# rockcarry/ffcnn

Measured on AMD Instinct MI355X. Metric: frames/sec yolo-fastest-1.1 @320x320 batch-64 per GPU (u8 BGR frames -> net_input's conversion in the first kernel -> full forward: conv stack + YOLO decode + NMS, boxes on rank 0), higher is better.
Workload: dtype f32

## Files before the change

ffcnn_amd/capi.py:

```python
import ctypes as C
import os
import subprocess

import numpy as np

HERE = os.path.dirname(os.path.abspath(__file__))
ROOT = os.path.dirname(HERE)
DATA = os.path.join(ROOT, "data")
CFG = os.path.join(DATA, "yolo-fastest-1.1.cfg")
WEIGHTS = os.path.join(DATA, "yolo-fastest-1.1.weights")

f32p = C.POINTER(C.c_float)


class FFGPU:
    MAX_DET = 128
    MERGE_LDS_SLOTS = 1024
    KEEP_ALL, COMPAT_V6, NO_GRAPH, NO_FUSE, HOST_DETS, SPLIT2, CONCURRENT, BF16_PW = 1, 2, 4, 8, 16, 32, 64, 128
    FEAT_FLAT, FEAT_MEAN, FEAT_MAX = 0, 1, 2
    POST_NONE, POST_SOFTMAX, POST_L2 = 0, 1, 2
    TOPK_MAX = 16
    RELABEL_KEEP_SCORE, RELABEL_LABEL_SCORE = 0, 1
    RELABEL_ENTRIES, RELABEL_MERGED = 0, 1
    K_AUTO, K_GENERIC, K_DW_STREAM, K_DW_LDS, K_PW_MFMA, K_PW_GEMM, _K6, K_DENSE_SMALL, K_IGEMM, K_PW_BF16, K_GROUP_THIN, K_PW_X3, K_CONV_X3, K_PW_X3T = range(14)
# ... 74 lines not shown


class Label(C.Structure):
    _fields_ = [("index", C.c_int), ("value", C.c_float)]


class RelabelSpec(C.Structure):
    _fields_ = [("min_value", C.c_float), ("type_base", C.c_int), ("score_mode", C.c_int), ("reserved", C.c_int)]


class Gallery(C.Structure):
    _fields_ = [("d_rows", C.c_void_p), ("d_ids", C.c_void_p), ("d_head", C.c_void_p), ("row_stride", C.c_long), ("capacity", C.c_int), ("d", C.c_int)]


class RedactSpec(C.Structure):
    _fields_ = [("mode", C.c_int), ("cell", C.c_int), ("flags", C.c_int), ("nclasses", C.c_int), ("classes", C.c_void_p), ("min_score", C.c_float),
                ("margin_num", C.c_int), ("margin_den", C.c_int), ("color", C.c_ubyte * 4)]


class Zone(C.Structure):
    _fields_ = [("x", C.c_float * 8), ("y", C.c_float * 8), ("nverts", C.c_int), ("dwell_frames", C.c_int), ("classes", C.c_uint * 4), ("reserved", C.c_int * 2)]


class Line(C.Structure):
    _fields_ = [("ax", C.c_float), ("ay", C.c_float), ("bx", C.c_float), ("by", C.c_float), ("classes", C.c_uint * 4)]


class Scene(C.Structure):
    _fields_ = [("zone", Zone * 8), ("line", Line * 8), ("nzones", C.c_int), ("nlines", C.c_int), ("anchor", C.c_int), ("reserved", C.c_int)]


class ZonesSpec(C.Structure):
    _fields_ = [("capacity", C.c_int), ("max_missed", C.c_int), ("identity", C.c_int), ("flags", C.c_int), ("min_score", C.c_float),
                ("gate_zone", C.c_uint), ("gate_line", C.c_uint), ("reserved", C.c_int)]


class ZoneSlot(C.Structure):
    _fields_ = [("id", C.c_int), ("px", C.c_float), ("py", C.c_float), ("inside", C.c_int), ("last", C.c_int), ("reserved", C.c_int * 3), ("since", C.c_int * 8)]


SCENE_ZONES, SCENE_LINES, ZONE_VERTS, ZONES_DETS, ZONES_ROW = 8, 8, 8, 128, 64
ZONES_NONE, ZONES_TYPE, ZONES_IDS = 0, 1, 2
ZONES_GATE_INVERT = 1
ZONES_ENTRIES, ZONES_MERGED = 0, 1
ZONES_EVENTS_HEADER = ("considered", "known", "fresh", "refused", "duplicate", "anonymous", "dropped", "freed", "live", "frame")
ZONES_STATE_HEADER = 144
TRACK_DETS = 128
TRACK_ENTRIES, TRACK_MERGED = 0, 1
TRACK_IDS_HEADER = ("considered", "matched", "born", "refused", "dropped", "freed", "live", "frame")
CROP_F32, CROP_U8 = 0, 1
CROP_ENTRIES, CROP_MERGED = 0, 1
REDACT_FILL, REDACT_MOSAIC = 0, 1
REDACT_OUTSIDE = 1
REDACT_ENTRIES, REDACT_MERGED = 0, 1
DRAW_ENTRIES, DRAW_MERGED = 0, 1
YUV_BT601_LIMITED, YUV_BT601_FULL, YUV_BT709_LIMITED, YUV_BT709_FULL = 0, 1, 2, 3

assert C.sizeof(LAYER) == 120 and C.sizeof(NET) == 104 and C.sizeof(BBOX) == 24
assert C.sizeof(FrameDets) == 16 + 24 * FFGPU.MAX_DET
assert C.sizeof(BgrFrame) == 24 and C.sizeof(Nv12Frame) == 40 and C.sizeof(Tile) == 16 and C.sizeof(TileRect) == 16
assert C.sizeof(DrawStyle) == 24 and C.sizeof(CropSpec) == 72 and C.sizeof(Crop) == 48
assert C.sizeof(TrackSpec) == 32 and C.sizeof(Track) == 48
assert C.sizeof(FeatureSpec) == 16 and C.sizeof(Label) == 8 and C.sizeof(RelabelSpec) == 16
assert C.sizeof(Gallery) == 40 and C.sizeof(RedactSpec) == 40
assert C.sizeof(Zone) == 96 and C.sizeof(Line) == 32 and C.sizeof(Scene) == 1040 and C.sizeof(ZonesSpec) == 32 and C.sizeof(ZoneSlot) == 64

BOX_DTYPE = np.dtype([("type", "<i4"), ("score", "<f4"), ("x1", "<f4"), ("y1", "<f4"), ("x2", "<f4"), ("y2", "<f4")])
DETS_DTYPE = np.dtype([("count", "<i4"), ("ncand", "<i4"), ("overflow", "<i4"), ("nfull", "<i4"),
                       ("box", BOX_DTYPE, (FFGPU.MAX_DET,))])
CROP_DTYPE = np.dtype([("target", "<i4"), ("box", "<i4"), ("type", "<i4"), ("score", "<f4"), ("x0", "<i4"), ("y0", "<i4"), ("w", "<i4"), ("h", "<i4"),
                       ("sw", "<i4"), ("sh", "<i4"), ("s1", "<i4"), ("s2", "<i4")])
TRACK_DTYPE = np.dtype([("id", "<i4"), ("type", "<i4"), ("score", "<f4"), ("x1", "<f4"), ("y1", "<f4"), ("x2", "<f4"), ("y2", "<f4"),
                        ("hits", "<i4"), ("missed", "<i4"), ("born", "<i4"), ("det", "<i4"), ("reserved", "<i4")])
ZONE_SLOT_DTYPE = np.dtype([("id", "<i4"), ("px", "<f4"), ("py", "<f4"), ("inside", "<i4"), ("last", "<i4"), ("reserved", "<i4", (3,)), ("since", "<i4", (8,))])
LABEL_DTYPE = np.dtype([("index", "<i4"), ("value", "<f4")])

EXPORTS = ["net_load", "net_free", "net_input", "net_forward", "net_dump", "net_profile", "groupconv",
           "ffgpu_device_count", "ffgpu_set_device", "ffgpu_last_error", "ffgpu_build_info",
           "ffgpu_net_weights_dev", "ffgpu_net_weights_commit",
           "ffgpu_exec_create", "ffgpu_exec_destroy", "ffgpu_exec_batch", "ffgpu_exec_arena_bytes",
           "ffgpu_exec_kernel_count", "ffgpu_exec_work_model", "ffgpu_exec_set_scale", "ffgpu_exec_forward_dev", "ffgpu_exec_forward_host",
           "ffgpu_exec_forward_bgr_dev", "ffgpu_exec_forward_bgr_frames_dev", "ffgpu_exec_forward_nv12_frames_dev", "ffgpu_exec_dets_dev", "ffgpu_exec_dets_host", "ffgpu_exec_set_ring", "ffgpu_exec_set_ring_strided", "ffgpu_exec_read_dets", "ffgpu_exec_read_layer", "ffgpu_exec_hash_layers",
           "ffgpu_exec_read_boxes", "ffgpu_exec_cand_capacity", "ffgpu_exec_graph_captures",
           "ffgpu_exec_profile", "ffgpu_exec_profile_steps", "ffgpu_exec_step_model", "ffgpu_groupconv_dev", "ffgpu_groupconv_kernel_name", "ffgpu_groupconv_time_dev", "ffgpu_irb_dev", "ffgpu_irb_plan_text", "ffgpu_irb_instantiations", "ffgpu_knobs_text", "ffgpu_dwpw_dev", "ffgpu_packed_records_bytes", "ffgpu_pack_records", "ffgpu_unpack_records",
           "ffgpu_shard_range", "ffgpu_node_create", "ffgpu_node_destroy", "ffgpu_node_ndev", "ffgpu_node_shard", "ffgpu_node_set_scale",
           "ffgpu_node_input_dev", "ffgpu_node_input_slot_dev", "ffgpu_node_depth", "ffgpu_node_rccl_ranks", "ffgpu_node_forward", "ffgpu_node_forward_host",
           "ffgpu_node_submit", "ffgpu_node_wait", "ffgpu_node_run",
           "ffgpu_merge_tiles_scratch_bytes", "ffgpu_merge_tiles_dev", "ffgpu_exec_merge_tiles", "ffgpu_exec_merged_dev", "ffgpu_exec_read_merged",
           "ffgpu_exec_read_merged_boxes", "ffgpu_tile_plan",
           "ffgpu_draw_boxes_bgr_dev", "ffgpu_draw_boxes_nv12_dev", "ffgpu_exec_draw_bgr", "ffgpu_exec_draw_nv12",
           "ffgpu_crop_table_bytes", "ffgpu_crop_slot_bytes", "ffgpu_crop_boxes_bgr_dev", "ffgpu_crop_boxes_nv12_dev", "ffgpu_exec_crop_bgr", "ffgpu_exec_crop_nv12",
           "ffgpu_crops_to_source_dev",
           "ffgpu_track_state_bytes", "ffgpu_track_reset_dev", "ffgpu_track_boxes_dev", "ffgpu_exec_track",
           "ffgpu_feature_dim", "ffgpu_exec_feature_dim", "ffgpu_features_dev", "ffgpu_exec_features", "ffgpu_topk_dev", "ffgpu_crops_relabel_dev",
           "ffgpu_exec_relabel",
           "ffgpu_match_workspace_bytes", "ffgpu_match_dev", "ffgpu_gallery_enroll_dev",
           "ffgpu_redact_boxes_bgr_dev", "ffgpu_redact_boxes_nv12_dev", "ffgpu_exec_redact_bgr", "ffgpu_exec_redact_nv12",
           "ffgpu_zones_state_bytes", "ffgpu_scene_check", "ffgpu_zones_reset_dev", "ffgpu_zones_boxes_dev", "ffgpu_exec_zones"]
DIAG_EXPORTS = ["ffgpu_membench", "ffgpu_pipe_probe", "ffgpu_pipe_probe2", "ffgpu_pipe_probe3", "ffgpu_mfma_floor", "ffgpu_diag_x3_term", "ffgpu_diag_xl_op", "ffgpu_clock_probe"]


def library_path():
    return os.environ.get("FFCNN_HIP_LIB") or os.path.join(HERE, "lib", "libffcnn_hip.so")


def build_library(force=False):
    cmd = ["make", "-C", os.path.join(HERE, "csrc")]
    if force:
        subprocess.check_call(cmd + ["clean"], stdout=subprocess.DEVNULL)
    subprocess.check_call(cmd, stdout=subprocess.DEVNULL)
    return library_path()


_lib = None


def lib():
    global _lib
    if _lib is not None:
        return _lib
    path = library_path()
    if not os.path.exists(path):
        raise RuntimeError("%s is missing: run `python -c 'import __graft_entry__ as g; g.build()'` "
                           "(the HIP extension is the only compute path)" % path)
    L = C.CDLL(path)
    vp, i, sz = C.c_void_p, C.c_int, C.c_size_t
    L.net_load.restype = C.POINTER(NET)
    L.net_load.argtypes = [C.c_char_p, C.c_char_p, i, i]
    L.net_free.argtypes = [C.POINTER(NET)]
    L.net_input.argtypes = [C.POINTER(NET), vp, i, i, f32p, f32p]
    L.net_forward.argtypes = [C.POINTER(NET)]
    L.net_dump.argtypes = [C.POINTER(NET)]
    L.net_profile.argtypes = [C.POINTER(NET)]
    L.groupconv.argtypes = [f32p, f32p, f32p] + [i] * 12 + [C.POINTER(f32p), C.POINTER(i)]
    L.ffgpu_last_error.restype = C.c_char_p
    L.ffgpu_build_info.restype = C.c_char_p
    if b" DIAG " in L.ffgpu_build_info() and os.environ.get("FFCNN_HIP_ALLOW_DIAG") != "1":
        raise RuntimeError("%s is a DIAG (lab) build of libffcnn_hip; set FFCNN_HIP_ALLOW_DIAG=1 to load it on purpose" % path)
    L.ffgpu_set_device.argtypes = [i]
    L.ffgpu_net_weights_dev.argtypes = [C.POINTER(NET), C.POINTER(vp), C.POINTER(sz)]
    L.ffgpu_net_weights_commit.argtypes = [C.POINTER(NET), vp]
    L.ffgpu_exec_create.restype = vp
    L.ffgpu_exec_create.argtypes = [C.POINTER(NET), i, i]
    L.ffgpu_exec_destroy.argtypes = [vp]
    L.ffgpu_exec_batch.argtypes = [vp]
    L.ffgpu_exec_arena_bytes.restype = sz
    L.ffgpu_exec_arena_bytes.argtypes = [vp]
    L.ffgpu_exec_kernel_count.argtypes = [vp]
    L.ffgpu_exec_work_model.argtypes = [vp, C.POINTER(C.c_double), C.POINTER(C.c_double)]
    L.ffgpu_exec_set_scale.argtypes = [vp, i, i]
    L.ffgpu_exec_forward_dev.argtypes = [vp, vp, vp]
    L.ffgpu_exec_forward_host.argtypes = [vp, f32p]
    L.ffgpu_exec_forward_bgr_dev.argtypes = [vp, vp, i, i, f32p, f32p, vp]
    L.ffgpu_exec_forward_bgr_frames_dev.argtypes = [vp, C.POINTER(BgrFrame), i, f32p, f32p, vp]
    L.ffgpu_exec_forward_nv12_frames_dev.argtypes = [vp, C.POINTER(Nv12Frame), i, f32p, f32p, vp]
    L.ffgpu_exec_dets_dev.argtypes = [vp, C.POINTER(vp), C.POINTER(sz)]
    L.ffgpu_exec_dets_host.restype = vp; L.ffgpu_exec_dets_host.argtypes = [vp]
    L.ffgpu_exec_set_ring.argtypes = [vp, vp, C.c_int]
    L.ffgpu_exec_set_ring_strided.argtypes = [vp, vp, C.c_int, C.c_int]
    L.ffgpu_exec_read_dets.argtypes = [vp, vp, i]
    L.ffgpu_exec_read_layer.argtypes = [vp, i, i, f32p, sz]
    L.ffgpu_exec_hash_layers.argtypes = [vp, vp, i]
    L.ffgpu_exec_profile.argtypes = [vp, vp, f32p]
    L.ffgpu_exec_profile_steps.argtypes = [vp, vp, C.POINTER(i), f32p, i]
    L.ffgpu_exec_step_model.argtypes = [vp, C.POINTER(i), C.POINTER(C.c_double), i]
    L.ffgpu_groupconv_dev.argtypes = [vp, vp, vp] + [i] * 15 + [vp]
    L.ffgpu_groupconv_kernel_name.restype = C.c_char_p
    L.ffgpu_groupconv_kernel_name.argtypes = [i] * 10
    L.ffgpu_groupconv_time_dev.restype = C.c_float
    L.ffgpu_groupconv_time_dev.argtypes = [vp, vp, vp] + [i] * 17 + [vp]
    L.ffgpu_irb_dev.restype = C.c_float
    L.ffgpu_irb_dev.argtypes = [vp] * 6 + [i] * 13 + [vp]
    L.ffgpu_irb_plan_text.argtypes = [i] * 12 + [C.c_char_p, i]
    L.ffgpu_irb_instantiations.argtypes = [C.c_char_p, i]
    L.ffgpu_knobs_text.argtypes = [C.c_char_p, i]
    L.ffgpu_exec_read_boxes.argtypes = [vp, i, vp, i]
    L.ffgpu_exec_cand_capacity.argtypes = [vp]
    L.ffgpu_exec_graph_captures.argtypes = [vp]
    L.ffgpu_dwpw_dev.restype = C.c_float
    L.ffgpu_dwpw_dev.argtypes = [vp] * 4 + [i] * 10 + [vp]
    L.ffgpu_packed_records_bytes.restype = C.c_size_t
    L.ffgpu_packed_records_bytes.argtypes = [i, i]
    L.ffgpu_pack_records.restype = i
    L.ffgpu_pack_records.argtypes = [vp, i, C.c_long, i, i, vp, vp]
    L.ffgpu_shard_range.argtypes = [i, i, i, C.POINTER(i), C.POINTER(i)]
    L.ffgpu_shard_range.restype = None
    L.ffgpu_node_create.restype = vp
    L.ffgpu_node_create.argtypes = [C.POINTER(NET), i, C.POINTER(i), i, i, i]
    L.ffgpu_node_destroy.argtypes = [vp]
    L.ffgpu_node_ndev.argtypes = [vp]
    L.ffgpu_node_shard.argtypes = [vp, i, C.POINTER(i), C.POINTER(i), C.POINTER(i)]
    L.ffgpu_node_set_scale.argtypes = [vp, i, i]
    L.ffgpu_node_input_dev.restype = vp
    L.ffgpu_node_input_dev.argtypes = [vp, i]
    L.ffgpu_node_input_slot_dev.restype = vp
    L.ffgpu_node_input_slot_dev.argtypes = [vp, i, i]
    L.ffgpu_node_depth.argtypes = [vp]
    if hasattr(L, "ffgpu_node_rccl_ranks"):
        L.ffgpu_node_rccl_ranks.argtypes = [vp]
    L.ffgpu_node_submit.restype = C.c_long
    L.ffgpu_node_submit.argtypes = [vp, f32p]
    L.ffgpu_node_wait.argtypes = [vp, C.c_long, vp]
    L.ffgpu_node_run.argtypes = [vp, C.c_long, vp]
    L.ffgpu_unpack_records.argtypes = [vp, i, i, vp]
    L.ffgpu_node_forward.argtypes = [vp, vp]
    L.ffgpu_node_forward_host.argtypes = [vp, f32p, vp]
    L.ffgpu_merge_tiles_scratch_bytes.restype = sz
    L.ffgpu_merge_tiles_scratch_bytes.argtypes = [i, i]
    L.ffgpu_merge_tiles_dev.argtypes = [vp, vp, i, C.POINTER(Tile), i, i, C.c_float, i, vp, vp, vp, sz, vp]
    L.ffgpu_exec_merge_tiles.argtypes = [vp, C.POINTER(Tile), i, i, vp]
    L.ffgpu_exec_merged_dev.argtypes = [vp, C.POINTER(vp), C.POINTER(sz)]
    L.ffgpu_exec_read_merged.argtypes = [vp, vp, i]
    L.ffgpu_exec_read_merged_boxes.argtypes = [vp, i, vp, i]
    L.ffgpu_tile_plan.argtypes = [i] * 7 + [C.POINTER(TileRect), i]
    L.ffgpu_draw_boxes_bgr_dev.argtypes = [vp, vp, i, C.POINTER(i), C.POINTER(BgrFrame), i, C.POINTER(DrawStyle), vp]
    L.ffgpu_draw_boxes_nv12_dev.argtypes = [vp, vp, i, C.POINTER(i), C.POINTER(Nv12Frame), i, C.POINTER(DrawStyle), vp]
    L.ffgpu_exec_draw_bgr.argtypes = [vp, i, C.POINTER(BgrFrame), i, C.POINTER(DrawStyle), vp]
    L.ffgpu_exec_draw_nv12.argtypes = [vp, i, C.POINTER(Nv12Frame), i, C.POINTER(DrawStyle), vp]
    L.ffgpu_redact_boxes_bgr_dev.argtypes = [vp, vp, i, C.POINTER(i), C.POINTER(BgrFrame), i, C.POINTER(RedactSpec), vp]
    L.ffgpu_redact_boxes_nv12_dev.argtypes = [vp, vp, i, C.POINTER(i), C.POINTER(Nv12Frame), i, C.POINTER(RedactSpec), vp]
    L.ffgpu_exec_redact_bgr.argtypes = [vp, i, C.POINTER(BgrFrame), i, C.POINTER(RedactSpec), vp]
    L.ffgpu_exec_redact_nv12.argtypes = [vp, i, C.POINTER(Nv12Frame), i, C.POINTER(RedactSpec), vp]
    L.ffgpu_crop_table_bytes.restype = sz
    L.ffgpu_crop_table_bytes.argtypes = [i]
    L.ffgpu_crop_slot_bytes.restype = sz
    L.ffgpu_crop_slot_bytes.argtypes = [i, i, i]
    L.ffgpu_crop_boxes_bgr_dev.argtypes = [vp, vp, i, C.POINTER(i), C.POINTER(BgrFrame), i, C.POINTER(CropSpec), vp, vp, i, vp]
    L.ffgpu_crop_boxes_nv12_dev.argtypes = [vp, vp, i, C.POINTER(i), C.POINTER(Nv12Frame), i, C.POINTER(CropSpec), vp, vp, i, vp]
    L.ffgpu_exec_crop_bgr.argtypes = [vp, i, C.POINTER(BgrFrame), i, C.POINTER(CropSpec), vp, vp, i, vp]
    L.ffgpu_exec_crop_nv12.argtypes = [vp, i, C.POINTER(Nv12Frame), i, C.POINTER(CropSpec), vp, vp, i, vp]
    L.ffgpu_crops_to_source_dev.argtypes = [vp, i, vp, vp, i, vp, vp, vp]
    L.ffgpu_track_state_bytes.restype = sz
    L.ffgpu_track_state_bytes.argtypes = [i, i]
    L.ffgpu_track_reset_dev.argtypes = [vp, i, i, i, vp]
    L.ffgpu_track_boxes_dev.argtypes = [vp, vp, i, C.POINTER(i), C.POINTER(i), i, C.POINTER(TrackSpec), vp, i, vp, vp, vp, vp]
    L.ffgpu_exec_track.argtypes = [vp, i, C.POINTER(i), i, C.POINTER(TrackSpec), vp, i, vp, vp, vp, vp]
    L.ffgpu_zones_state_bytes.restype = sz
    L.ffgpu_zones_state_bytes.argtypes = [i, i]
    L.ffgpu_scene_check.argtypes = [C.POINTER(Scene), i]
    L.ffgpu_zones_reset_dev.argtypes = [vp, i, i, i, vp]
    L.ffgpu_zones_boxes_dev.argtypes = [vp, vp, i, C.POINTER(i), C.POINTER(i), i, C.POINTER(ZonesSpec), vp, vp, i, vp, vp, vp, vp, vp]
    L.ffgpu_exec_zones.argtypes = [vp, i, C.POINTER(i), i, C.POINTER(ZonesSpec), vp, vp, i, vp, vp, vp, vp, vp]
    L.ffgpu_feature_dim.argtypes = [i, i, i, i]
    L.ffgpu_exec_feature_dim.argtypes = [vp, C.POINTER(FeatureSpec)]
    L.ffgpu_features_dev.argtypes = [vp, i, i, i, i, i, i, vp, C.c_long, vp]
    L.ffgpu_exec_features.argtypes = [vp, C.POINTER(FeatureSpec), vp, C.c_long, vp]
    L.ffgpu_topk_dev.argtypes = [vp, i, i, C.c_long, i, vp, vp]
    L.ffgpu_crops_relabel_dev.argtypes = [vp, i, vp, i, vp, vp, i, C.POINTER(i), i, C.POINTER(RelabelSpec), vp, vp, vp]
    L.ffgpu_exec_relabel.argtypes = [vp, i, vp, i, vp, i, i, C.POINTER(RelabelSpec), vp, vp, vp]
    L.ffgpu_match_workspace_bytes.restype = sz
    L.ffgpu_match_workspace_bytes.argtypes = [i, i, i]
    L.ffgpu_match_dev.argtypes = [vp, i, C.c_long, C.POINTER(Gallery), i, vp, vp, C.c_long, vp, sz, vp]
    L.ffgpu_gallery_enroll_dev.argtypes = [C.POINTER(Gallery), vp, i, C.c_long, vp, i, C.c_float, vp, vp]
    _lib = L
    return L

# ... 729 lines not shown
        _check(lib().ffgpu_node_run(self.h, steps, out.ctypes.data), "ffgpu_node_run")
        return out

    def input_slot_dev(self, rank, slot):
        return lib().ffgpu_node_input_slot_dev(self.h, rank, slot)

    def __init__(self, net, ndev, global_batch, devices=None, exec_flags=0, node_flags=0):
        self.net, self.ndev, self.total = net, ndev, global_batch
        dv = (C.c_int * ndev)(*devices) if devices is not None else None
        self.h = lib().ffgpu_node_create(net.p, ndev, dv, global_batch, exec_flags, node_flags)
        if not self.h:
            raise RuntimeError("ffgpu_node_create failed: %s" % last_error())

    def close(self):
        if self.h:
            lib().ffgpu_node_destroy(self.h)
            self.h = None

    def __enter__(self):
        return self

    def __exit__(self, *a):
        self.close()

    def shard(self, rank):
        lo, hi, dev = C.c_int(), C.c_int(), C.c_int()
        _check(lib().ffgpu_node_shard(self.h, rank, C.byref(lo), C.byref(hi), C.byref(dev)), "ffgpu_node_shard")
        return lo.value, hi.value, dev.value

    def set_scale(self, s1, s2):
        _check(lib().ffgpu_node_set_scale(self.h, s1, s2), "ffgpu_node_set_scale")

    def input_dev(self, rank):
        return lib().ffgpu_node_input_dev(self.h, rank)

    def forward(self):
        out = np.zeros(self.total, DETS_DTYPE)
        _check(lib().ffgpu_node_forward(self.h, out.ctypes.data), "ffgpu_node_forward")
        return out

    def forward_host(self, frames):
        frames = np.ascontiguousarray(frames, np.float32)
        assert frames.shape == (self.total,) + self.net.input_shape, frames.shape
        out = np.zeros(self.total, DETS_DTYPE)
        _check(lib().ffgpu_node_forward_host(self.h, frames.ctypes.data_as(f32p), out.ctypes.data), "ffgpu_node_forward_host")
        return out


def groupconv_dev(d_in, d_filt, d_out, batch, iw, ih, ic, groups, pad, stride, fs, fn, act=0, flags=0, variant=0, stream=None):
    ow, oh = (iw + 2 * pad - fs) // stride + 1, (ih + 2 * pad - fs) // stride + 1
    _check(lib().ffgpu_groupconv_dev(d_in, d_filt, d_out, batch, iw, ih, ic, groups, pad, stride, fs, fn, ow, oh, fn,
                                     act, flags, variant, stream), "ffgpu_groupconv_dev")


def groupconv_time_dev(d_in, d_filt, d_out, batch, iw, ih, ic, groups, pad, stride, fs, fn, act=0, flags=0, variant=0,
                       warmup=5, iters=20, stream=None):
    ow, oh = (iw + 2 * pad - fs) // stride + 1, (ih + 2 * pad - fs) // stride + 1
    us = lib().ffgpu_groupconv_time_dev(d_in, d_filt, d_out, batch, iw, ih, ic, groups, pad, stride, fs, fn, ow, oh, fn,
                                        act, flags, variant, warmup, iters, stream)
    if us < 0:
        raise RuntimeError("ffgpu_groupconv_time_dev failed: %s" % last_error())
    return us


def packed_records_bytes(batch, cap):
    return int(lib().ffgpu_packed_records_bytes(batch, cap))


def pack_records_dev(d_records, nslots, slot_stride_records, batch, cap, d_out, stream=None):
    _check(lib().ffgpu_pack_records(d_records, nslots, slot_stride_records, batch, cap, d_out, stream), "ffgpu_pack_records")


def kernel_name(batch, iw, ih, ic, groups, pad, stride, fs, fn, variant=0):
    return lib().ffgpu_groupconv_kernel_name(batch, iw, ih, ic, groups, pad, stride, fs, fn, variant).decode()


def irb_plan_text(shape, flags=0):
    buf = C.create_string_buffer(1024)
    if lib().ffgpu_irb_plan_text(*shape, flags, buf, len(buf)) < 0:
        raise RuntimeError("ffgpu_irb_plan_text failed: %s" % last_error())
    return buf.value.decode()


def irb_instantiations():
    buf = C.create_string_buffer(4096)
    n = lib().ffgpu_irb_instantiations(buf, len(buf))
    if n < 0 or n >= len(buf):
        raise RuntimeError("ffgpu_irb_instantiations failed: %s" % (last_error() if n < 0 else "%d bytes" % n))
    return buf.value.decode().split()


def knobs():
    buf = C.create_string_buffer(1 << 16)
    n = lib().ffgpu_knobs_text(buf, len(buf))
    if n < 0 or n >= len(buf):
        raise RuntimeError("ffgpu_knobs_text failed: %s" % (last_error() if n < 0 else "%d bytes" % n))
    rows = []
    for line in buf.value.decode().splitlines():
        name, kind, dflt, cls, value, text = line.split(" ", 5)
        rows.append({"name": name, "kind": kind, "default": None if dflt == "-" else dflt if dflt == "computed" else int(dflt), "cls": cls, "value": value, "text": text})
    return rows


def dwpw_dev(d_in, d_wd, d_wp, d_out, batch, iw, ih, c, oc, fs, actd=2, actp=0, warmup=0, iters=0, stream=None):
    us = lib().ffgpu_dwpw_dev(d_in, d_wd, d_wp, d_out, batch, iw, ih, c, oc, fs, actd, actp, warmup, iters, stream)
    if us < 0:
        raise RuntimeError("ffgpu_dwpw_dev failed: %s" % last_error())
    return us


def irb_dev(d_in, d_w1, d_wd, d_w2, d_res, d_out, batch, iw, ih, ic, ec, oc, stride, act1=2, actd=2, act2=0, res_act=0,
            warmup=0, iters=0, stream=None):
    us = lib().ffgpu_irb_dev(d_in, d_w1, d_wd, d_w2, d_res, d_out, batch, iw, ih, ic, ec, oc, stride, act1, actd, act2, res_act,
                             warmup, iters, stream)
    if us < 0:
        raise RuntimeError("ffgpu_irb_dev failed: %s" % last_error())
    return us
```

ffcnn_amd/csrc/ffgpu_conv_kernels.inc:

```
#include "ffgpu_dw_stream.inc"
#include "ffgpu_pw_mfma.inc"
#include "ffgpu_pw_gemm32.inc"
#include "ffgpu_pw_bf16.inc"
#include "ffgpu_conv_igemm.inc"
#include "ffgpu_dwpw.inc"
#include "ffgpu_conv_dense.inc"
#include "ffgpu_irb.inc"
#include "ffgpu_irb_thin.inc"
#include "ffgpu_front.inc"
#include "ffgpu_irb_wave.inc"
#include "ffgpu_irb_wave2.inc"
#include "ffgpu_pw_x3.inc"
#include "ffgpu_pw_x3t.inc"
#include "ffgpu_conv_x3.inc"
#include "ffgpu_dw_lds.inc"
#include "ffgpu_dw_pair.inc"
#include "ffgpu_conv_thin.inc"

struct BareScratch {
    float *p = nullptr; size_t n = 0; int dev = -1;
    float *get(size_t need)
    {
        int d = 0;
        (void)hipGetDevice(&d);
        if (p && dev == d && n >= need) return p;
        if (p) (void)hipFree(p);
        p = nullptr; n = 0; dev = d;
        if (hipMalloc(&p, need * sizeof(float)) != hipSuccess) { p = nullptr; return nullptr; }
        n = need;
        return p;
    }
};

static int device_cus()
{
    static int cu_of[64];
    static std::mutex cu_mu;
    int dev = 0, cus = 0;
    (void)hipGetDevice(&dev);
    std::lock_guard<std::mutex> lk(cu_mu);
    if (dev >= 0 && dev < 64) {
        if (!cu_of[dev]) (void)hipDeviceGetAttribute(&cu_of[dev], hipDeviceAttributeMultiprocessorCount, dev);
        cus = cu_of[dev];
    } else (void)hipDeviceGetAttribute(&cus, hipDeviceAttributeMultiprocessorCount, dev);
    return cus > 0 ? cus : 256;
}

static unsigned umulhi_magic(long dv) { return dv == 1 ? 0u : (unsigned)(((1ULL << 32) + (unsigned long long)dv - 1) / (unsigned long long)dv); }

static void split_main_narrow(long P, int ntm, int slots, bool narrow_on, long *ntn_main, long *ntn_narrow)
{
    const long ntn_all = (P + 127) / 128, total_all = ntn_all * ntm;
    long tail_tiles = total_all % slots;
    if (total_all <= slots / 2) tail_tiles = total_all;
    else if (tail_tiles > slots * 5 / 8) tail_tiles = 0;
    if (!narrow_on) tail_tiles = 0;
    const long tail_ntn = (tail_tiles + ntm - 1) / ntm;
    *ntn_main = ntn_all - tail_ntn;
    const long npx_narrow = P - *ntn_main * 128;
    *ntn_narrow = npx_narrow > 0 ? (npx_narrow + 63) / 64 : 0;
}

static bool conv_cnhw_contiguous(const ConvDesc &d)
{
    return d.in_ns == (long)d.iw * d.ih && d.in_cs == (long)d.N * d.iw * d.ih &&
           d.out_ns == (long)d.ow * d.oh && d.out_cs == (long)d.N * d.ow * d.oh &&
           (!d.residual || (d.res_ns == d.out_ns && d.res_cs == d.out_cs));
}
static bool conv_is_depthwise(const ConvDesc &d) { return d.groups == d.ic && d.ic == d.oc; }
static bool conv_is_pointwise(const ConvDesc &d) { return d.fs == 1 && d.stride == 1 && d.pad == 0 && d.groups == 1; }

static bool dw_stream_ok(const ConvDesc &d)
{
    return conv_is_depthwise(d) && d.fs == 3 && d.stride == 1 && d.pad == 1 && conv_cnhw_contiguous(d) &&
           d.iw % 4 == 0 && d.iw >= 40 && d.iw <= 512 && d.ih >= 2 && !d.residual && d.act != 3;
}
static bool pw_mfma_ok(const ConvDesc &d)
{
    const long P = (long)d.N * d.iw * d.ih;
    return conv_is_pointwise(d) && conv_cnhw_contiguous(d) && P % 4 == 0 && ((d.ic + 3) & ~3) <= 1024 && P < (1L << 28);
}

static int pw_x3_mt(const ConvDesc &d) { const int f = knob(K_PWX3_MT); return f == 4 || f == 2 || f == 1 ? f : 4; }
static bool pw_x3_ok(const ConvDesc &d)
{
    const long P = (long)d.N * d.iw * d.ih;
    return pw_mfma_ok(d) && (long)(d.ic + 32) * P < (1L << 30);
}
static bool pw_x3_auto(const ConvDesc &d)
{
    const long P = (long)d.N * d.iw * d.ih;
    return pw_x3_ok(d) && d.ic >= knob(K_PWX3_MIN_IC) && d.oc >= knob(K_PWX3_MIN_OC) && P >= knob(K_PWX3_MIN_P) &&
           knob(K_PW_X3) != 0;
}
// ... 1352 lines not shown
size_t ffgpu_irb_pack_floats(const IrbDesc &d) { return irb_planned(d, "irb_pack_floats") ? (size_t)d.plan.pack_floats : 0; }

int ffgpu_irb_pack(const IrbDesc &d, float *pk, hipStream_t s)
{
    const IrbPlan &c = d.plan;
    if (!irb_planned(d, "irb_pack")) return -1;
    if (c.family == IRB_THIN) return 0;
    if (c.family == IRB_WAVE) {
        IrbwPackP q; q.w1 = d.w1; q.wd = d.wd; q.w2 = d.w2; q.pk = pk; q.ic = d.ic; q.ec = d.ec; q.oc = d.oc;
        q.k4 = (d.ic + 3) & ~3; q.OT = c.OT; q.ngroups = c.ngroups; q.x3 = c.x3; q.half = c.half;
        hipLaunchKernelGGL(k_irbw_pack, dim3((c.pack_floats + 255) / 256), dim3(256), 0, s, q);
        LAUNCH_OK("irbw_pack");
        return 0;
    }
    IrbPackP q;
    q.w1 = d.w1; q.wd = d.wd; q.w2 = d.w2; q.pk = pk;
    q.ic = d.ic; q.ec = d.ec; q.oc = d.oc;
    q.k4 = (d.ic + 3) & ~3; q.ECH = c.ECH; q.MT = c.ECH / 16; q.OT = c.OT; q.nchunks = (d.ec + c.ECH - 1) / c.ECH; q.CH = irb_chunk_floats(q.k4, c.ECH, c.OT);
    const int total = q.nchunks * q.CH + q.OT * 32;
    hipLaunchKernelGGL(k_irb_pack, dim3((total + 255) / 256), dim3(256), 0, s, q);
    LAUNCH_OK("irb_pack");
    return 0;
}

static int irb_thin_key(int ic, int oc, char *key, size_t cap) { return snprintf(key, cap, "thin<%d,8,%d>", ic, oc); }
static int irbw_key(const IrbwKernel &k, char *key, size_t cap)
{
    if (k.NSO == 2) return snprintf(key, cap, "irbw2<%d,%d%s>", k.KS1, k.NSI, k.x3 ? ",x3" : "");
    return snprintf(key, cap, "irbw<%d,%d,%d,%d%s%s%s>", k.KS1, k.OT, k.S, k.NSI, k.big ? ",big" : "", k.x3 ? ",x3" : "", k.xl ? ",xl" : "");
}
static int irb_key(const IrbKernel &k, char *key, size_t cap) { return snprintf(key, cap, "irb<%d,%d,%d,%d,%d>", k.MT, k.OT, k.S, k.NW == 8 ? 1 : 2, k.NW); }

int ffgpu_irb_keys(char *buf, size_t cap)
{
    size_t n = 0;
    char key[48];
    auto put = [&]() { n += (size_t)snprintf(n < cap ? buf + n : nullptr, n < cap ? cap - n : 0, "%s\n", key); };
    for (const IrbThinKernel &k : irb_thin_kernels) { irb_thin_key(k.IC, k.OC, key, sizeof key); put(); }
    for (const IrbwKernel &k : irbw_kernels) { irbw_key(k, key, sizeof key); put(); }
    for (const IrbKernel &k : irb_kernels) { irb_key(k, key, sizeof key); put(); }
    return (int)n;
}

int ffgpu_irb_plan_line(const IrbDesc &d, char *buf, size_t cap)
{
    const IrbPlan &c = d.plan;
    char key[48];
    if (c.family == IRB_THIN) {
        const ThinP p = thin_params(d);
        irb_thin_key(d.ic, d.oc, key, sizeof key);
        return snprintf(buf, cap, "%s W=%d H=%d N=%d band=%d nbands=%d act=%g,%g,%g,%g ntasks=%ld lds=%d grid=%d block=%d half=%d pack=%d",
                        key, p.W, p.H, p.N, p.band, p.nbands, p.act1, p.actd, p.act2, p.res_act, p.ntasks, c.lds, c.grid, c.block, c.half, c.pack_floats);
    }
    if (c.family == IRB_WAVE) {
        const IrbwP p = irbw_params(d);
        const IrbwKernel &k = irbw_kernels[c.inst];
        irbw_key(k, key, sizeof key);
        return snprintf(buf, cap, "%s N=%d H=%d W=%d OH=%d OW=%d ic=%d ec=%d oc=%d act=%g,%g,%g,%g tile=%d,%d,%d,%d tiles=%d,%d,%ld ngroups=%d G=%d WPB=%d o_w2=%d o_cs=%d cs_floats=%d "
                        "xl_off=%d red_cap=%d in_elems=%u vec=%d half_last=%d m=%u,%u,%u,%u xcd=%d lds=%d grid=%d block=%d half=%d pack=%d",
                        key, p.N, p.H, p.W, p.OH, p.OW, p.ic, p.ec, p.oc, p.act1, p.actd, p.act2, p.res_act, p.TWq, p.TH, p.EW, p.EH, p.tiles_x, p.tiles_y, p.ntiles, p.ngroups, p.G, p.WPB,
                        p.o_w2, p.o_cs, p.cs_floats, p.xl_off, p.red_cap, p.in_elems, p.vec, p.half_last, p.m_ew, p.m_tx, p.m_ty, p.m_twq, p.xcd, c.lds, c.grid, c.block, c.half, c.pack_floats);
    }
    if (c.family == IRB_WG) {
        const IrbP p = irb_params(d);
        const IrbKernel &k = irb_kernels[c.inst];
        irb_key(k, key, sizeof key);
        return snprintf(buf, cap, "%s N=%d H=%d W=%d OH=%d OW=%d ic=%d ec=%d oc=%d stride=%d act=%g,%g,%g,%g tile=%d,%d,%d,%d,%d,%d NPin=%d NPout=%d tiles=%d,%d,%d "
                        "k4=%d nchunks=%d ECH=%d CH=%d KS=%d red_off=%d vec_store=%d resident=%d inv_nsi=%d lds=%d grid=%d block=%d half=%d pack=%d",
                        key, p.N, p.H, p.W, p.OH, p.OW, p.ic, p.ec, p.oc, p.stride, p.act1, p.actd, p.act2, p.res_act, p.TH, p.TW, p.TWq, p.NF, p.EH, p.EW,
                        p.NPin, p.NPout, p.tiles_x, p.tiles_y, p.ntiles, p.k4, p.nchunks, p.ECH, p.CH, p.KS, p.red_off, p.vec_store, p.resident, p.inv_nsi, c.lds, c.grid, c.block, c.half, c.pack_floats);
    }
    return snprintf(buf, cap, "unsupported");
}

int ffgpu_launch_irb(const IrbDesc &d, hipStream_t s)
{
    const IrbPlan &c = d.plan;
    if (!irb_planned(d, "irb")) return -1;
    if (knob(K_VERBOSE_IRB)) { char line[1024]; ffgpu_irb_plan_line(d, line, sizeof line); fprintf(stderr, "%s\n", line); }
    if (c.family == IRB_THIN) return launch_irb_thin(d, s);
    if (!d.pk) { ffgpu_set_error("irb: constants not packed"); return -1; }
    return c.family == IRB_WAVE ? irbw_kernels[c.inst].launch(irbw_params(d), c, s) : irb_kernels[c.inst].launch(irb_params(d), c, s);
}
```

ffcnn_amd/csrc/ffgpu_dev.hpp:

```cpp
#pragma once
#include <hip/hip_runtime.h>
#include <stddef.h>
#include <stdint.h>
#include <vector>
#include "ffgpu_internal.h"
#include "ffgpu_args.hpp"
#include "ffgpu_zones_host.hpp"

#define FFGPU_CHECK(expr)                                                                   \
    do {                                                                                    \
        hipError_t e_ = (expr);                                                             \
        if (e_ != hipSuccess) {                                                             \
            ffgpu_set_error("%s failed: %s (%s:%d)", #expr, hipGetErrorString(e_), __FILE__, __LINE__); \
            return -1;                                                                      \
        }                                                                                   \
    } while (0)

struct ConvDesc {
    const float *in;
    const float *const *in_ind;
    const float *filt;
    float       *out;
    const float *residual;
    const float *wpack;
    int   N;
    int   iw, ih, ic;
    int   ow, oh, oc;
    int   fs, stride, pad, groups;
    int   act;
    int   res_act;
    int   flags;
    long  in_cs, in_ns, out_cs, out_ns, res_cs, res_ns;
    int   nsplit;
    int   kernel;
    int   x3_mt;
};
#define FFGPU_F_BATCH_INPUT (1 << 30)

static inline int conv_k4(const ConvDesc &d) { return (d.fs * d.fs * (d.ic / d.groups) + 3) & ~3; }

enum { IRB_NONE = 0, IRB_THIN, IRB_WAVE, IRB_WG };
struct IrbPlan {
    int family;
    int inst;
    int half;
    int pack_floats;
    int lds, grid, block;
    int KS1, OT, NSI, NSO, TWq, TH, EW, EH, ngroups, G, WPB, big, x3, xl;
    int xcd, region;
    int TW, NF, ECH, NW, KS, wbufs, red_off;
    int band, front_band;
};
struct IrbDesc {
    const float *in; float *out; const float *residual;
    const float *w1, *wd, *w2;
    int N, H, W, OH, OW, ic, ec, oc, stride;
    int act1, actd, act2, res_act;
    const float *pk;
    int flags;
    IrbPlan plan;
};
bool   ffgpu_irb_plan(IrbDesc &d);
size_t ffgpu_irb_pack_floats(const IrbDesc &d);
int    ffgpu_irb_pack(const IrbDesc &d, float *pk, hipStream_t s);
int    ffgpu_launch_irb(const IrbDesc &d, hipStream_t s);
int    ffgpu_irb_plan_line(const IrbDesc &d, char *buf, size_t cap);
int    ffgpu_irb_keys(char *buf, size_t cap);
bool   ffgpu_front_ok(const ConvDesc &c, const IrbDesc &d);
enum InputForm { IN_F32, IN_U8, IN_BGR_FRAMES, IN_NV12_FRAMES, IN_FORMS };
int    ffgpu_launch_front(const ConvDesc &c, const IrbDesc &d, InputForm form, hipStream_t s);
bool   ffgpu_front_nv12_fused();
int    ffgpu_front_nc(const IrbDesc &d);

bool   ffgpu_dwpw_ok(const ConvDesc &dw, const ConvDesc &pw);
size_t ffgpu_dwpw_pack_floats(const ConvDesc &dw, const ConvDesc &pw);
int    ffgpu_dwpw_pack(const ConvDesc &dw, const ConvDesc &pw, float *pk, hipStream_t s);
int    ffgpu_launch_dwpw(const ConvDesc &dw, const ConvDesc &pw, const float *wpack, hipStream_t s);

size_t ffgpu_pw_pack_floats(const ConvDesc &d);
void   ffgpu_conv_plan(ConvDesc &d);
int    ffgpu_pw_pack(const ConvDesc &d, float *pk, hipStream_t s);

#define FFGPU_YUV_MATRICES { { 16, 298, 409, 100, 208, 516 }, { 0, 256, 359, 88, 183, 454 }, { 16, 298, 459, 55, 136, 541 }, { 0, 256, 403, 48, 120, 475 } }
int  ffgpu_launch_set_frames(FrameDesc *d_tab, const FrameDesc *h_desc, int n, hipStream_t s);
int  ffgpu_launch_input_frames(const FrameDesc *d_tab, bool nv12, float *out, int N, int W, int H, const float mean[3], const float norm[3], hipStream_t s);

struct ExecParams {
    const float *frames;
    int s1, s2;
    ffgpu_frame_dets *ring;
    int ring_slots, ring_stride;
    int bbox_max;
    const unsigned char *bgr;
    long  bgr_frame;
    int   bgr_pitch;
    float mean[3], norm[3];
    const FrameDesc *frames_tab;
};
int  ffgpu_launch_set_params(ExecParams *d_prm, const ExecParams &v, hipStream_t s);
bool ffgpu_conv_supports_ind(const ConvDesc &d);

bool ffgpu_no_device(const char *what);

int         ffgpu_launch_conv(const ConvDesc &d, int variant, hipStream_t s);
const char *ffgpu_conv_kernel_name(const ConvDesc &d, int variant);
int ffgpu_launch_pool(const float *in, float *out, int N, int c, int w, int h, int fs, int stride, int is_max, hipStream_t s);
int ffgpu_launch_spp(const float *in, float *const out[3], const int fs[3], int n, long planes, int w, int h, hipStream_t s);
int ffgpu_launch_upsample(const float *in, float *out, long planes, int w, int h, int stride, hipStream_t s);
int ffgpu_launch_add_act(const float *a, const float *b, float *out, long n, int act, hipStream_t s);
int ffgpu_launch_copy(const float *src, float *dst, long n, hipStream_t s);
int ffgpu_launch_hash64(const float *x, long n, unsigned long long *out, hipStream_t s);
int ffgpu_launch_input_bgr(const unsigned char *bgr, float *out, int N, int w, int h, int W, int H,
                           int sw, int sh, int s1, int s2, const float mean[3], const float norm[3], hipStream_t s);

struct YoloHead {
    const float *in;
    int   w, h, classes;
    int   anchors[3][2];
    float thresh, scale_xy;
    int   key_base;
};
int ffgpu_launch_yolo(const YoloHead &hd, int N, int netw, int neth, BBOX *cand, int *cand_key, int *ncand, int cap, int *ring_ctr, hipStream_t s);
int ffgpu_launch_nms(const BBOX *cand, const int *cand_key, int *ncand, int cap, BBOX *full, void *scratch,
                     ffgpu_frame_dets *dets, ffgpu_frame_dets *dets_host, const int *ring_ctr, int N,
                     float thresh, int use_min, const ExecParams *prm, hipStream_t s);
#define FFGPU_NMS_LDS_CAP 8192
bool ffgpu_nms_in_lds(int cap_pow2);
int ffgpu_launch_clear(int *ncand, int N, int *ring_ctr, hipStream_t s);

int    ffgpu_merge_build_tab(const char *what, const ffgpu_tile *tiles, int ntiles, int nimages, std::vector<int> &tab, std::vector<int> *off);
size_t ffgpu_merge_tab_bytes(int ntiles);
int    ffgpu_launch_set_ints(int *d_dst, const int *h_src, int n, hipStream_t s);
int    ffgpu_launch_merge_tiles(const int *d_tab, const std::vector<int> &tab, const ffgpu_frame_dets *recs, const BBOX *lists, int stride,
                                float thresh, int use_min, ffgpu_frame_dets *out_recs, BBOX *out_lists, void *scratch, hipStream_t s);

int ffgpu_draw_style_check(const char *what, const ffgpu_draw_style *st, unsigned pal[256], int *npal);
int ffgpu_launch_draw(bool nv12, const DetSource &src, const std::vector<DrawTarget> &targets, const unsigned pal[256], int npal, int thickness, hipStream_t s);

struct CropPlan {
    int   out_w, out_h, form, per_target, nclasses, num, den;
    float min_score, mean[3], norm[3];
    unsigned char classes[256];
};
int ffgpu_box_sel_check(const char *what, int nclasses, const unsigned char *classes, int margin_num, int margin_den);
int ffgpu_crop_spec_check(const char *what, const ffgpu_crop_spec *sp, CropPlan &pl);
int ffgpu_crop_buffers_check(const char *what, const void *d_out, const void *d_table, int capacity);
int ffgpu_launch_crop(bool nv12, const DetSource &src, const std::vector<CropSrc> &sources, const CropPlan &pl, void *d_out, void *d_table, int capacity, hipStream_t s);

struct RedactPlan {
    int   mode, cell, outside, nclasses, num, den;
// ... 21 lines not shown
```

ffcnn_amd/csrc/ffgpu_exec.hip:

```cpp
#include <algorithm>
#include <cstdarg>
#include <cstdint>
#include <cstdio>
#include <cstdlib>
#include <cstring>
#include <map>
#include <mutex>
#include <string>
#include <type_traits>
#include <vector>

#include "ffgpu_dev.hpp"
#include "ffgpu_knobs.hpp"
#include "ffgpu_plan.hpp"
#include "conv.h"

static thread_local char g_err[512] = "";

extern "C" void ffgpu_set_error(const char *fmt, ...)
{
    va_list ap;
    va_start(ap, fmt);
    vsnprintf(g_err, sizeof g_err, fmt, ap);
    va_end(ap);
// ... 17 lines not shown
    if (hipGetDeviceCount(&n) != hipSuccess) { (void)hipGetLastError(); return 0; }
    return n;
}

bool ffgpu_no_device(const char *what)
{
    if (ffgpu_device_count() > 0) return false;
    ffgpu_set_error("%s: no HIP device visible: libffcnn_hip has no CPU fallback", what);
    return true;
}

extern "C" int ffgpu_set_device(int ordinal)
{
    FFGPU_CHECK(hipSetDevice(ordinal));
    return 0;
}

namespace {
struct PinnedRange { const char *p; size_t bytes; };
std::mutex g_pin_mu;
std::vector<PinnedRange> g_pinned;

bool pinned_ours(const void *ptr, size_t bytes)
{
    const char *c = static_cast<const char *>(ptr);
    std::lock_guard<std::mutex> lk(g_pin_mu);
    for (const PinnedRange &r : g_pinned) if (c >= r.p && c + bytes <= r.p + r.bytes) return true;
    return false;
}

constexpr size_t BOUNCE_BYTES = (size_t)16 << 20;
struct Bounce { std::mutex mu; char *p = nullptr; };
Bounce g_bounces[32];

Bounce &bounce_cur()
{
    int dev = 0;
    (void)hipGetDevice(&dev);
    return g_bounces[(unsigned)dev % 32u];
}

int bounce_ready(Bounce &b)
{
    if (b.p) return 0;
    FFGPU_CHECK(hipHostMalloc((void **)&b.p, BOUNCE_BYTES, hipHostMallocPortable));
    return 0;
}
}

static int copy_h2d(void *d_dst, const void *h_src, size_t bytes)
{
    if (bytes == 0) return 0;
    if (pinned_ours(h_src, bytes)) { FFGPU_CHECK(hipMemcpy(d_dst, h_src, bytes, hipMemcpyHostToDevice)); return 0; }
    Bounce &bn = bounce_cur();
    std::lock_guard<std::mutex> lk(bn.mu);
    if (bounce_ready(bn)) return -1;
    char *const g_bounce = bn.p;
    for (size_t off = 0; off < bytes; off += BOUNCE_BYTES) {
        const size_t n = std::min(BOUNCE_BYTES, bytes - off);
        memcpy(g_bounce, static_cast<const char *>(h_src) + off, n);
        FFGPU_CHECK(hipMemcpy(static_cast<char *>(d_dst) + off, g_bounce, n, hipMemcpyHostToDevice));
    }
    return 0;
}

static int copy_d2h(void *h_dst, const void *d_src, size_t bytes)
{
    if (bytes == 0) return 0;
    if (pinned_ours(h_dst, bytes)) { FFGPU_CHECK(hipMemcpy(h_dst, d_src, bytes, hipMemcpyDeviceToHost)); return 0; }
    Bounce &bn = bounce_cur();
    std::lock_guard<std::mutex> lk(bn.mu);
    if (bounce_ready(bn)) return -1;
    char *const g_bounce = bn.p;
    for (size_t off = 0; off < bytes; off += BOUNCE_BYTES) {
        const size_t n = std::min(BOUNCE_BYTES, bytes - off);
        FFGPU_CHECK(hipMemcpy(g_bounce, static_cast<const char *>(d_src) + off, n, hipMemcpyDeviceToHost));
        memcpy(static_cast<char *>(h_dst) + off, g_bounce, n);
    }
    return 0;
}

#define FFGPU_INTERNAL_CHILD 0x40000000

enum StepKind { S_CONV, S_POOL, S_UPSAMPLE, S_ADD, S_COPY, S_YOLO, S_NMS, S_CLEAR, S_TOCNHW, S_IRB, S_FRONT, S_DWPW };

struct Step {
    StepKind kind;
    int      layer;
    int      ltype;
    ConvDesc conv;
    ConvDesc conv2;
    bool     in_is_input;
    bool     b_is_input;
    const float *a, *b;
    float   *out;
    long     n;
    int      w, h, c, fs, stride, flag;
    YoloHead head;
    IrbDesc  irb;
    float   *out2[2];
    int      fs2[2];
    int      lane;
};

struct ffgpu_netdev {
    NET   *net = nullptr;
    std::mutex mu;
    std::vector<ffgpu_exec *> execs;
    double us_acc[LAYER_TYPE_TOTOAL] = {};
    float *d_weights = nullptr;
    size_t weight_bytes = 0;
    int    device = 0;
    ffgpu_exec *exec1 = nullptr;
};

struct InputSrc {
    InputForm form;
    const float *frames;
    const unsigned char *bgr; long bgr_frame; int bgr_pitch;
    const FrameDesc *ftab;
    float mean[3], norm[3];
    InputSrc slice(int c, int part_frames, size_t part_floats) const
    {
        InputSrc p = *this;
        if (frames) p.frames = frames + c * part_floats;
        if (bgr) p.bgr = bgr + (long)c * part_frames * bgr_frame;
        if (ftab) p.ftab = ftab + (size_t)c * part_frames;
        return p;
    }
};
static InputSrc fp32_src(const float *d_frames) { InputSrc in = {}; in.frames = d_frames; return in; }
static InputSrc u8_src(InputForm form, const float mean[3], const float norm[3])
{
    InputSrc in = {};
    in.form = form;
    for (int k = 0; k < 3; k++) { in.mean[k] = mean[k]; in.norm[k] = norm[k]; }
    return in;
}

struct ffgpu_exec {
    NET *net = nullptr;
    ffgpu_netdev *dev = nullptr;
    int  N = 1, flags = 0, device = 0;
    int  in_c = 0, in_h = 0, in_w = 0;
    std::vector<Step>   steps;
    NetLayout layout;
    float *arena = nullptr;
    float *d_input = nullptr;
    float *d_pack = nullptr;
    BBOX  *d_cand = nullptr;
    int   *d_cand_key = nullptr, *d_ncand = nullptr;
    int    cand_cap = 1, bbox_max = 1;
    BBOX  *d_full = nullptr;
    void  *d_nms_scratch = nullptr;
    ExecParams *d_prm = nullptr;
    bool   indirect = false;
    ExecParams prm_sent = {}; hipStream_t prm_stream = nullptr; bool prm_valid = false;
    InputSrc last = {};
    ffgpu_frame_dets *d_dets = nullptr;
    ffgpu_frame_dets *h_dets = nullptr, *h_dets_dev = nullptr;
    FrameDesc *d_ftab = nullptr;
    std::vector<FrameDesc> ftab_sent; hipStream_t ftab_stream = nullptr;
    float *h_stage = nullptr;
    ffgpu_frame_dets *d_merged = nullptr; BBOX *d_merged_full = nullptr; void *d_merge_scratch = nullptr; int *d_mtab = nullptr;
    std::vector<int> mtab_sent, mrg_off; hipStream_t mtab_stream = nullptr;
    ffgpu_frame_dets *ring = nullptr; int ring_slots = 0; int *d_ringctr = nullptr;
    int ring_stride = 0;
    static constexpr int MAXPART = 8;
    ffgpu_exec *child[MAXPART] = {};
    int nchild = 0;
    hipStream_t part_stream[MAXPART] = {}; hipEvent_t part_ev[MAXPART] = {};
    bool is_child = false;
    int    s1 = 1, s2 = 1;
    hipStream_t own_stream = nullptr, last_stream = nullptr;
    hipStream_t side_stream = nullptr;
    hipEvent_t  ev_fork = nullptr, ev_join = nullptr;
    hipGraphExec_t graph[IN_FORMS] = {};
    struct Keyed { const float *in; hipGraphExec_t g; unsigned long stamp; };
    std::vector<Keyed> graphs;
    unsigned long graph_stamp = 0;
    int captures = 0;
    int kernel_count = 0;
};

static float *tensor_ptr(const ffgpu_exec *ex, int t) { return ex->arena + ex->layout.offset_of(t); }

static PlanOptions plan_options(const ffgpu_exec *ex)
{
    PlanOptions o;
    o.batch = ex->N;
    o.keep_all = ex->flags & FFGPU_KEEP_ALL;
    o.fuse = !(ex->flags & FFGPU_NO_FUSE);
    o.branch = knob(K_BRANCH) && !ex->is_child;
    o.no_irb = knob(K_NO_IRB); o.irb_min_ec = knob(K_IRB_MIN_EC);
    o.dwpw = knob(K_DWPW);
    return o;
}

static ConvDesc layer_desc(const ffgpu_exec *ex, int i, int flag_mask = FFGPU_COMPAT_V6)
{
    ConvDesc d{};
    const LAYER &a = ex->net->layer_list[i], &b = ex->net->layer_list[i + 1];
    const int N = ex->N;
    d.N = N; d.iw = a.w; d.ih = a.h; d.ic = a.c; d.ow = b.w; d.oh = b.h; d.oc = b.c;
    d.fs = a.fs; d.stride = a.stride; d.pad = a.pad; d.groups = a.groups; d.act = a.activation;
    d.flags = ex->flags & flag_mask;
    d.in_cs = (long)N * a.w * a.h; d.in_ns = (long)a.w * a.h;
    d.out_cs = (long)N * b.w * b.h; d.out_ns = (long)b.w * b.h;
    return d;
}

static IrbDesc irb_desc(const ffgpu_exec *ex, int p0)
{
    IrbDesc d{};
    const LAYER *ll = ex->net->layer_list;
    const LAYER &a = ll[p0], &b = ll[p0 + 1], &c = ll[p0 + 2];
    const int sc = ex->layout.fused_into[p0 + 2];
    d.N = ex->N; d.H = a.h; d.W = a.w; d.OH = ll[p0 + 3].h; d.OW = ll[p0 + 3].w;
    d.ic = a.c; d.ec = a.fn; d.oc = c.fn; d.stride = b.stride; d.flags = ex->flags & FFGPU_CONCURRENT;
    d.act1 = a.activation; d.actd = b.activation; d.act2 = c.activation;
    d.res_act = sc >= 0 ? ll[sc].activation : 0;
    return d;
}

static int plan_layout(ffgpu_exec *ex, std::vector<IrbDesc> &irb_planned)
{
    const PlanOptions opt = plan_options(ex);
    irb_planned.assign(ex->net->layer_num, IrbDesc{});
    auto block_ok = [&](int p0) {
        IrbDesc d = irb_desc(ex, p0);
        if (!ffgpu_irb_plan(d) || (d.ec < opt.irb_min_ec && d.plan.family != IRB_THIN)) return false;
        irb_planned[p0 + 2] = d;
        return true;
    };
    auto pair_ok = [&](int p0) { return ffgpu_dwpw_ok(layer_desc(ex, p0), layer_desc(ex, p0 + 1)); };
    return ffgpu_net_layout(ex->net->layer_list, ex->net->layer_num, opt, block_ok, pair_ok, ex->layout);
}

static int plan_arena(ffgpu_exec *ex)
{
    const size_t bytes = ex->layout.arena_floats * sizeof(float);
    if (hipMalloc(&ex->arena, bytes) != hipSuccess) { ffgpu_set_error("arena hipMalloc(%zu bytes) failed", bytes); return -1; }
    return 0;
}

static int plan_steps(ffgpu_exec *ex, const std::vector<IrbDesc> &irb_planned)
{
    const NetLayout &nl = ex->layout;
    const LAYER *ll = ex->net->layer_list;
    const int L = ex->net->layer_num, N = ex->N;
    std::vector<Step> &S = ex->steps;
    S.clear();
    { Step c{}; c.kind = S_CLEAR; c.layer = -1; c.ltype = LAYER_TYPE_YOLO; S.push_back(c); }
    int key_base = 0;
    float *cnhw_input = nullptr;
    bool bad_chain = false;
    auto ptr = [&](int t) { return tensor_ptr(ex, t); };
    auto weights = [&](int i) { return ex->dev->d_weights + (ll[i].filter - ex->net->weight_buf); };
    auto in_ptr = [&](int i, bool *is_input) -> const float * {
        const int t = nl.src(i - 1);
        *is_input = t == -1;
        if (t < -1) bad_chain = true;
        return t >= 0 ? ptr(t) : nullptr;
    };
    for (int i = 0; i < L; i++) {
        const LAYER &a = ll[i];
        Step st{};
        st.layer = i; st.ltype = a.type;
        bool from_input = false;
        switch (a.type) {
        case LAYER_TYPE_CONV: {
            if (nl.canon[i] == -3) break;
            if (nl.irb_tail[i] >= 0) {
                const int p0 = nl.irb_tail[i];
                IrbDesc &d = st.irb = irb_planned[i];
                st.kind = S_IRB;
                d.in = ptr(nl.src(p0 - 1));
                d.out = ptr(nl.canon[i]);
                d.w1 = weights(p0); d.wd = weights(p0 + 1); d.w2 = weights(p0 + 2);
                if (nl.fused_into[i] >= 0) d.residual = ptr(nl.src(ll[nl.fused_into[i]].depend_list[0]));
            } else if (nl.dwpw_tail[i] >= 0) {
                const int p0 = nl.dwpw_tail[i];
                st.kind = S_DWPW;
                st.conv = layer_desc(ex, p0); st.conv2 = layer_desc(ex, i);
                st.conv.in = ptr(nl.src(p0 - 1));
                st.conv.filt = weights(p0); st.conv2.filt = weights(i);
                st.conv2.out = ptr(nl.canon[i]);
            } else {
                ConvDesc &d = st.conv = layer_desc(ex, i, FFGPU_COMPAT_V6 | FFGPU_BF16_PW);
                st.kind = S_CONV;
                d.in = in_ptr(i, &st.in_is_input);
                d.filt = weights(i);
                d.out = ptr(nl.canon[i]);
                if (st.in_is_input) { d.in_cs = (long)a.w * a.h; d.in_ns = (long)a.c * a.w * a.h; }
                if (nl.fused_into[i] >= 0) {
                    const LAYER &sc = ll[nl.fused_into[i]];
                    d.residual = ptr(nl.src(sc.depend_list[0]));
                    d.res_act = sc.activation; d.res_cs = d.out_cs; d.res_ns = d.out_ns;
                }
            }
            S.push_back(st);
            break; }
        case LAYER_TYPE_AVGPOOL: case LAYER_TYPE_MAXPOOL: case LAYER_TYPE_UPSAMPLE: case LAYER_TYPE_SHORTCUT: {
            const float *src = in_ptr(i, &from_input);
            const bool b_input = a.type == LAYER_TYPE_SHORTCUT && nl.src(a.depend_list[0]) == -1;
            if (a.type == LAYER_TYPE_SHORTCUT && nl.src(a.depend_list[0]) < -1) { bad_chain = true; break; }
            if ((from_input || b_input) && N > 1) {
                if (!cnhw_input) {
                    const LAYER &l0 = ll[0];
                    if (hipMalloc(&cnhw_input, (size_t)l0.w * l0.h * l0.c * N * sizeof(float)) != hipSuccess) { ffgpu_set_error("hipMalloc failed"); return -1; }
                    Step cv{}; cv.kind = S_TOCNHW; cv.layer = -1; cv.ltype = a.type; cv.out = cnhw_input; cv.c = l0.c; cv.w = l0.w; cv.h = l0.h; cv.in_is_input = true;
                    S.push_back(cv);
                }
                if (from_input) { src = cnhw_input; from_input = false; }
            }
            st.in_is_input = from_input;
            st.a = src;
            if (a.type == LAYER_TYPE_SHORTCUT) {
                if (nl.canon[i - 1] == i) break;
                st.kind = S_ADD;
                st.b = b_input ? cnhw_input : ptr(nl.src(a.depend_list[0]));
                st.b_is_input = b_input && N == 1;
                st.out = ptr(nl.canon[i]);
                st.n = (long)ll[i + 1].w * ll[i + 1].h * ll[i + 1].c * N; st.flag = a.activation;
            } else {
                st.kind = a.type == LAYER_TYPE_UPSAMPLE ? S_UPSAMPLE : S_POOL;
                st.out = ptr(nl.canon[i]);
                st.c = a.c; st.w = a.w; st.h = a.h; st.fs = a.fs; st.stride = a.stride;
                st.flag = a.type == LAYER_TYPE_MAXPOOL;
            }
            S.push_back(st);
            break; }
        case LAYER_TYPE_ROUTE: {
            if (nl.canon[i] != i || nl.route_inplace[i]) break;
            long off = 0;
            for (int k = 0; k < a.depend_num; k++) {
                const int t = nl.src(a.depend_list[k]);
                if (t < 0) { ffgpu_set_error("route %d: unsupported source", i); return -1; }
                const LAYER &o = ll[a.depend_list[k] + 1];
                Step cp{}; cp.kind = S_COPY; cp.layer = i; cp.ltype = a.type;
                cp.a = ptr(t); cp.out = ptr(i) + off; cp.n = (long)o.w * o.h * o.c * N;
                S.push_back(cp);
                off += cp.n;
            }
            break; }
        case LAYER_TYPE_YOLO: {
            st.kind = S_YOLO;
            YoloHead &hd = st.head;
            hd.in = in_ptr(i, &from_input);
            if (from_input) { ffgpu_set_error("yolo head directly on the input is not supported"); return -1; }
            hd.w = a.w; hd.h = a.h; hd.classes = a.class_num;
            memcpy(hd.anchors, a.anchor_list, sizeof hd.anchors);
            hd.thresh = a.ignore_thres; hd.scale_xy = a.scale_x_y; hd.key_base = key_base;
            key_base += a.w * a.h * 3;
            S.push_back(st);
            break; }
        default: break;
        }
    }
    if (bad_chain) { ffgpu_set_error("a layer consumes the (non-existent) output of a yolo head"); return -1; }
    return 0;
}

static void fuse_front(ffgpu_exec *ex)
{
    std::vector<Step> &S = ex->steps;
    for (size_t k = 0; k + 1 < S.size(); k++) {
        Step &c0 = S[k];
        const Step &b0 = S[k + 1];
        if (c0.kind != S_CONV || b0.kind != S_IRB || c0.layer < 0 || ex->layout.nuses[c0.layer] != 1) continue;
        if (!ffgpu_front_ok(c0.conv, b0.irb)) continue;
        c0.kind = S_FRONT; c0.irb = b0.irb;
        ex->layout.readable[c0.layer] = 0;
        S.erase(S.begin() + k + 1);
        break;
    }
}

static void merge_spp(std::vector<Step> &S)
{
    for (size_t i = 0; i + 1 < S.size(); i++) {
        Step &a = S[i];
        if (a.kind != S_POOL || !a.flag || a.stride != 1 || a.in_is_input || (long)a.w * a.h > 8192) continue;
        int k = 0;
        while (k < 2 && i + 1 < S.size()) {
            const Step &b = S[i + 1];
            if (b.kind != S_POOL || !b.flag || b.stride != 1 || b.in_is_input || b.a != a.a || b.c != a.c || b.w != a.w || b.h != a.h) break;
            a.out2[k] = b.out; a.fs2[k] = b.fs; k++;
            S.erase(S.begin() + i + 1);
        }
    }
}

static void rewrite_steps(ffgpu_exec *ex)
{
    std::vector<Step> &S = ex->steps;
    const bool fuse = !(ex->flags & FFGPU_NO_FUSE);
    if (fuse) { fuse_front(ex); merge_spp(S); }
    const auto head = std::find_if(S.begin(), S.end(), [](const Step &t) { return t.kind == S_YOLO; });
    if (head != S.end() && fuse) {
        head->flag = 1;
        S.erase(std::remove_if(S.begin(), S.end(), [](const Step &t) { return t.kind == S_CLEAR; }), S.end());
    }
    { Step nm{}; nm.kind = S_NMS; nm.layer = -1; nm.ltype = LAYER_TYPE_YOLO; S.push_back(nm); }
    const NetLayout &nl = ex->layout;
    for (Step &st : S) st.lane = (nl.side_lo >= 0 && st.layer >= nl.side_lo && st.layer <= nl.side_hi) ? 1 : 0;
}

static size_t pack_floats(const Step &st)
{
    if (st.kind == S_IRB) return ffgpu_irb_pack_floats(st.irb);
    if (st.kind == S_DWPW) return ffgpu_dwpw_pack_floats(st.conv, st.conv2);
    if (st.kind == S_CONV) return ffgpu_pw_pack_floats(st.conv);
    return 0;
}

static int place_constants(ffgpu_exec *ex)
{
    size_t tot = 0;
    for (Step &st : ex->steps) {
        if (st.kind == S_CONV) {
            if (st.in_is_input) st.conv.flags |= FFGPU_F_BATCH_INPUT;
            ffgpu_conv_plan(st.conv);
        }
        tot += pack_floats(st);
    }
    if (!tot) return 0;
    if (hipMalloc(&ex->d_pack, tot * sizeof(float)) != hipSuccess) { ffgpu_set_error("hipMalloc(pack) failed"); return -1; }
    size_t off = 0;
    for (Step &st : ex->steps) {
        const size_t n = pack_floats(st);
        if (st.kind == S_IRB) st.irb.pk = ex->d_pack + off;
        else if (st.kind == S_DWPW) st.conv2.wpack = ex->d_pack + off;
        else if (st.kind == S_CONV && n) st.conv.wpack = ex->d_pack + off;
        off += n;
    }
    return 0;
}

static void decide_indirect(ffgpu_exec *ex)
{
    ex->indirect = !knob(K_NO_INDIRECT);
    for (const Step &st : ex->steps)
        if (st.b_is_input || (st.in_is_input && !(st.kind == S_FRONT || (st.kind == S_CONV && ffgpu_conv_supports_ind(st.conv))))) ex->indirect = false;
    if (ex->indirect)
        for (Step &st : ex->steps) if (st.in_is_input) st.conv.in_ind = reinterpret_cast<const float *const *>(ex->d_prm);
}

static int plan(ffgpu_exec *ex)
{
    std::vector<IrbDesc> irb_planned;
    if (plan_layout(ex, irb_planned) || plan_arena(ex) || plan_steps(ex, irb_planned)) return -1;
    rewrite_steps(ex);
    if (place_constants(ex)) return -1;
    decide_indirect(ex);
    ex->kernel_count = (int)ex->steps.size();
    return 0;
}

static int repack(ffgpu_exec *ex, hipStream_t s)
{
    for (const Step &st : ex->steps) {
        if (st.kind == S_IRB && ffgpu_irb_pack(st.irb, const_cast<float *>(st.irb.pk), s)) return -1;
        if (st.kind == S_DWPW && ffgpu_dwpw_pack(st.conv, st.conv2, const_cast<float *>(st.conv2.wpack), s)) return -1;
        if (st.kind == S_CONV && st.conv.wpack && ffgpu_pw_pack(st.conv, const_cast<float *>(st.conv.wpack), s)) return -1;
    }
    return 0;
}

static int issue_step(ffgpu_exec *ex, const Step &st, const InputSrc &in, hipStream_t s)
{
    const float *const d_frames = in.frames;
#ifdef FFGPU_DIAG
    if (knob_text(K_DBG_SKIP) || knob_text(K_DBG_KEEP)) {
        static bool warned = false;
        if (!warned) { warned = true; fprintf(stderr, "libffcnn_hip: FFGPU_DBG_SKIP / FFGPU_DBG_KEEP set -- launches are being dropped, RESULTS ARE WRONG (tuning only)\n"); }
    }
    if (const char *sk = knob_text(K_DBG_SKIP)) {
        int lo = -1, hi = -1;
        if (sscanf(sk, "%d:%d", &lo, &hi) == 2 && st.layer >= lo && st.layer <= hi && st.kind != S_NMS) return 0;
    }
    if (const char *sk = knob_text(K_DBG_KEEP)) {
        int lo = -1, hi = -1;
        if (sscanf(sk, "%d:%d", &lo, &hi) == 2 && (st.layer < lo || st.layer > hi) && st.kind != S_NMS) return 0;
    }
#endif
    switch (st.kind) {
    case S_CLEAR:
        return ffgpu_launch_clear(ex->d_ncand, ex->N, ex->d_ringctr, s);
    case S_CONV: {
        ConvDesc d = st.conv;
        if (st.in_is_input && !d.in_ind) d.in = d_frames;
        return ffgpu_launch_conv(d, FFGPU_K_AUTO, s); }
    case S_POOL:
        if (st.fs2[0]) {
            float *const outs[3] = { st.out, st.out2[0], st.out2[1] };
            const int fss[3] = { st.fs, st.fs2[0], st.fs2[1] };
            return ffgpu_launch_spp(st.a, outs, fss, st.fs2[1] ? 3 : 2, (long)ex->N * st.c, st.w, st.h, s);
        }
        return ffgpu_launch_pool(st.in_is_input ? d_frames : st.a, st.out, ex->N, st.c, st.w, st.h, st.fs, st.stride, st.flag, s);
    case S_UPSAMPLE:
        return ffgpu_launch_upsample(st.in_is_input ? d_frames : st.a, st.out, (long)ex->N * st.c, st.w, st.h, st.stride, s);
    case S_ADD:
        return ffgpu_launch_add_act(st.in_is_input ? d_frames : st.a, st.b_is_input ? d_frames : st.b, st.out, st.n, st.flag, s);
    case S_COPY:
        return ffgpu_launch_copy(st.a, st.out, st.n, s);
    case S_TOCNHW: {
        const long plane = (long)st.w * st.h;
        for (int c = 0; c < st.c; c++)
            FFGPU_CHECK(hipMemcpy2DAsync(st.out + (long)c * ex->N * plane, plane * sizeof(float),
                                         d_frames + (long)c * plane, (size_t)st.c * plane * sizeof(float),
                                         plane * sizeof(float), ex->N, hipMemcpyDeviceToDevice, s));
        return 0; }
    case S_IRB:
        return ffgpu_launch_irb(st.irb, s);
    case S_DWPW:
        return ffgpu_launch_dwpw(st.conv, st.conv2, st.conv2.wpack, s);
    case S_FRONT: {
        ConvDesc d = st.conv;
        if (st.in_is_input && !d.in_ind) d.in = d_frames;
        return ffgpu_launch_front(d, st.irb, in.form, s); }
    case S_YOLO:
        return ffgpu_launch_yolo(st.head, ex->N, ex->in_w, ex->in_h, ex->d_cand, ex->d_cand_key, ex->d_ncand, ex->cand_cap,
                                 st.flag ? ex->d_ringctr : nullptr, s);
    case S_NMS:
        return ffgpu_launch_nms(ex->d_cand, ex->d_cand_key, ex->d_ncand, ex->cand_cap, ex->d_full, ex->d_nms_scratch,
                                ex->d_dets, ex->h_dets_dev, ex->d_ringctr, ex->N, 0.5f, 1, ex->d_prm, s);
    }
    return -1;
}

static int issue_all(ffgpu_exec *ex, const InputSrc &in, hipStream_t s)
{
    bool forked = false, joined = true;
    for (const Step &st : ex->steps) {
        if (st.lane == 1) {
            if (!ex->side_stream) FFGPU_CHECK(hipStreamCreateWithFlags(&ex->side_stream, hipStreamNonBlocking));
            if (!forked) {
                FFGPU_CHECK(hipEventRecord(ex->ev_fork, s));
                FFGPU_CHECK(hipStreamWaitEvent(ex->side_stream, ex->ev_fork, 0));
                forked = true; joined = false;
            }
            if (issue_step(ex, st, in, ex->side_stream) != 0) return -1;
            continue;
        }
        if (st.kind == S_NMS && !joined) {
            FFGPU_CHECK(hipEventRecord(ex->ev_join, ex->side_stream));
            FFGPU_CHECK(hipStreamWaitEvent(s, ex->ev_join, 0));
            joined = true;
        }
        if (issue_step(ex, st, in, s) != 0) return -1;
    }
    if (!joined) {
        FFGPU_CHECK(hipEventRecord(ex->ev_join, ex->side_stream));
        FFGPU_CHECK(hipStreamWaitEvent(s, ex->ev_join, 0));
    }
    return 0;
}

static int issue_split(ffgpu_exec *ex, const InputSrc &in, hipStream_t s)
{
    const int pn = ex->child[0]->N;
    const size_t part = (size_t)pn * ex->in_c * ex->in_h * ex->in_w;
    FFGPU_CHECK(hipEventRecord(ex->ev_fork, s));
    for (int c = 1; c < ex->nchild; c++) FFGPU_CHECK(hipStreamWaitEvent(ex->part_stream[c], ex->ev_fork, 0));
    for (int c = 0; c < ex->nchild; c++)
        if (issue_all(ex->child[c], in.slice(c, pn, part), c ? ex->part_stream[c] : s) != 0) return -1;
    for (int c = 1; c < ex->nchild; c++) {
        FFGPU_CHECK(hipEventRecord(ex->part_ev[c], ex->part_stream[c]));
        FFGPU_CHECK(hipStreamWaitEvent(s, ex->part_ev[c], 0));
    }
    return 0;
}

static int push_params(ffgpu_exec *ex, const InputSrc &in, hipStream_t s)
{
    if (ex->child[0]) {
        const int pn = ex->child[0]->N;
        const size_t part = (size_t)pn * ex->in_c * ex->in_h * ex->in_w;
        for (int c = 0; c < ex->nchild; c++) {
            ffgpu_exec *ch = ex->child[c];
            ch->s1 = ex->s1; ch->s2 = ex->s2; ch->bbox_max = ex->bbox_max; ch->last_stream = s;
            if (push_params(ch, in.slice(c, pn, part), s)) return -1;
        }
        return 0;
    }
    ex->last = in;
    ExecParams v;
    memset(&v, 0, sizeof v);
    v.frames = in.frames; v.s1 = ex->s1; v.s2 = ex->s2;
    v.bgr = in.bgr; v.bgr_frame = in.bgr_frame; v.bgr_pitch = in.bgr_pitch;
    for (int k = 0; k < 3; k++) { v.mean[k] = in.mean[k]; v.norm[k] = in.norm[k]; }
    v.frames_tab = in.ftab;
    v.bbox_max = ex->bbox_max;
    v.ring = ex->ring; v.ring_slots = ex->ring_slots; v.ring_stride = ex->ring_stride ? ex->ring_stride : ex->N;
    if (ex->prm_valid && ex->prm_stream == s && memcmp(&v, &ex->prm_sent, sizeof v) == 0) return 0;
    if (ffgpu_launch_set_params(ex->d_prm, v, s)) return -1;
    ex->prm_sent = v; ex->prm_stream = s; ex->prm_valid = true;
// ... 138 lines not shown
    if (ok && (flags & FFGPU_HOST_DETS)) {
        ok = hipHostMalloc(&ex->h_dets, sizeof(ffgpu_frame_dets) * (size_t)batch, hipHostMallocMapped) == hipSuccess
          && hipHostGetDevicePointer((void **)&ex->h_dets_dev, ex->h_dets, 0) == hipSuccess;
        if (ok) memset(ex->h_dets, 0, sizeof(ffgpu_frame_dets) * (size_t)batch);
    }
    if (!ok) { ffgpu_set_error("executor buffers: %s", hipGetErrorString(hipGetLastError())); ffgpu_exec_destroy(ex); return nullptr; }
    ex->last_stream = ex->own_stream;
    if (split) {
        int K = 2;
        const int parts = knob(K_SPLIT_PARTS);
        if ((parts == 4 || parts == 8) && batch % parts == 0) K = parts;
        for (int c = 0; c < K; c++) {
            ffgpu_exec *ch = exec_create_on(dev, net, batch / K, (flags & ~FFGPU_HOST_DETS) | FFGPU_INTERNAL_CHILD);
            if (!ch) { ffgpu_exec_destroy(ex); return nullptr; }
            (void)hipFree(ch->d_dets); (void)hipFree(ch->d_full);
            ch->d_dets = ex->d_dets + (size_t)c * (batch / K);
            ch->d_full = ex->d_full + (size_t)c * (batch / K) * ex->cand_cap;
            ch->h_dets_dev = ex->h_dets_dev ? ex->h_dets_dev + (size_t)c * (batch / K) : nullptr;
            ex->child[c] = ch; ex->nchild = c + 1;
            ex->kernel_count += ch->kernel_count;
            ex->layout.arena_floats += ch->layout.arena_floats;
            if (c && (hipStreamCreateWithFlags(&ex->part_stream[c], hipStreamNonBlocking) != hipSuccess ||
                      hipEventCreateWithFlags(&ex->part_ev[c], hipEventDisableTiming) != hipSuccess)) {
                ffgpu_set_error("split executor: stream / event creation failed"); ffgpu_exec_destroy(ex); return nullptr; }
        }
        { std::lock_guard<std::mutex> lk(dev->mu); dev->execs.push_back(ex); }
        if (capture_at_create(ex)) { ffgpu_exec_destroy(ex); return nullptr; }
        return ex;
    }
    if (plan(ex) != 0 || repack(ex, ex->own_stream) != 0 || hipStreamSynchronize(ex->own_stream) != hipSuccess) { ffgpu_exec_destroy(ex); return nullptr; }
    { std::lock_guard<std::mutex> lk(dev->mu); dev->execs.push_back(ex); }
    if (!as_child && capture_at_create(ex)) { ffgpu_exec_destroy(ex); return nullptr; }
    return ex;
}

extern "C" void ffgpu_exec_destroy(ffgpu_exec *ex)
{
    if (!ex) return;
    int cur_dev = ex->device;
    (void)hipGetDevice(&cur_dev);
    if (cur_dev != ex->device) (void)hipSetDevice(ex->device);
    if (ex->last_stream) (void)hipStreamSynchronize(ex->last_stream);
    if (!ex->is_child) (void)hipDeviceSynchronize();
    for (int c = 0; c < ffgpu_exec::MAXPART; c++) {
        if (ex->child[c]) { ffgpu_exec_destroy(ex->child[c]); ex->child[c] = nullptr; }
        if (ex->part_stream[c]) (void)hipStreamDestroy(ex->part_stream[c]);
        if (ex->part_ev[c]) (void)hipEventDestroy(ex->part_ev[c]);
    }
    if (ex->is_child) { ex->d_dets = nullptr; ex->d_full = nullptr; }
    if (ex->dev) {
        std::lock_guard<std::mutex> lk(ex->dev->mu);
        ex->dev->execs.erase(std::remove(ex->dev->execs.begin(), ex->dev->execs.end(), ex), ex->dev->execs.end());
    }
    drop_graphs(ex);
    for (const Step &st : ex->steps) if (st.kind == S_TOCNHW) (void)hipFree(st.out);
    (void)hipFree(ex->arena); (void)hipFree(ex->d_input); (void)hipFree(ex->d_pack); (void)hipFree(ex->d_cand);
    (void)hipFree(ex->d_cand_key); (void)hipFree(ex->d_ncand); (void)hipFree(ex->d_dets);
    (void)hipFree(ex->d_full); (void)hipFree(ex->d_prm); (void)hipFree(ex->d_nms_scratch); (void)hipFree(ex->d_ftab);
    (void)hipFree(ex->d_merged); (void)hipFree(ex->d_merged_full); (void)hipFree(ex->d_merge_scratch); (void)hipFree(ex->d_mtab);
    if (ex->h_dets) (void)hipHostFree(ex->h_dets);
    if (ex->h_stage) (void)hipHostFree(ex->h_stage);
    (void)hipFree(ex->d_ringctr);
    if (ex->own_stream) (void)hipStreamDestroy(ex->own_stream);
    if (ex->side_stream) (void)hipStreamDestroy(ex->side_stream);
    if (ex->ev_fork) (void)hipEventDestroy(ex->ev_fork);
    if (ex->ev_join) (void)hipEventDestroy(ex->ev_join);
    if (cur_dev != ex->device) (void)hipSetDevice(cur_dev);
    delete ex;
}

extern "C" int ffgpu_exec_batch(const ffgpu_exec *ex) { return ex ? ex->N : 0; }
extern "C" size_t ffgpu_exec_arena_bytes(const ffgpu_exec *ex) { return ex ? ex->layout.arena_floats * sizeof(float) : 0; }
extern "C" int ffgpu_exec_kernel_count(const ffgpu_exec *ex) { return ex ? ex->kernel_count : 0; }

static double step_model_bytes(const ffgpu_exec *ex, const Step &st)
{
    const double N = ex->N;
    auto rows = [](const ConvDesc &d) { return (double)d.oc * (conv_k4(d) + 4); };
    switch (st.kind) {
    case S_CONV: { const ConvDesc &d = st.conv;
        return 4.0 * (N * d.ic * d.ih * d.iw + N * d.oc * d.oh * d.ow * (d.residual ? 2 : 1) + rows(d)); }
    case S_IRB: { const IrbDesc &d = st.irb;
        return 4.0 * (N * d.ic * d.H * d.W + N * d.oc * d.OH * d.OW * (d.residual ? 2 : 1) + (double)d.ec * (d.ic + 4 + 16) + (double)d.oc * (d.ec + 4)); }
    case S_DWPW: { const ConvDesc &a = st.conv, &b = st.conv2;
        return 4.0 * (N * a.ic * a.ih * a.iw + N * b.oc * b.oh * b.ow + rows(a) + rows(b)); }
    case S_FRONT: { const ConvDesc &c = st.conv; const IrbDesc &d = st.irb;
        return 4.0 * (N * c.ic * c.ih * c.iw + N * d.oc * d.OH * d.OW + rows(c)); }
    case S_POOL: { const int np = 1 + (st.fs2[0] != 0) + (st.fs2[1] != 0);
        return 4.0 * N * st.c * ((double)st.w * st.h + (double)np * (st.w / st.stride) * (st.h / st.stride)); }
    case S_UPSAMPLE: return 4.0 * N * st.c * (double)st.w * st.h * (1 + st.stride * st.stride);
    case S_ADD: return 4.0 * 3 * st.n;
    case S_COPY: return 4.0 * 2 * st.n;
    case S_TOCNHW: return 4.0 * 2 * N * st.c * (double)st.w * st.h;
    case S_YOLO: return 4.0 * N * 3 * (5 + st.head.classes) * (double)st.head.w * st.head.h;
    default: return 0.0;
    }
}

extern "C" int ffgpu_exec_step_model(const ffgpu_exec *ex, int *layer_of, double *hbm_bytes, int cap)
{
    if (!ex || !ex->net || !layer_of || !hbm_bytes) { ffgpu_set_error("step_model: bad argument"); return -1; }
    if (ex->child[0]) { ffgpu_set_error("step_model: not available on a split executor"); return -1; }
    const int n = (int)std::min<size_t>(ex->steps.size(), (size_t)(cap > 0 ? cap : 0));
    for (int i = 0; i < n; i++) { layer_of[i] = ex->steps[i].layer; hbm_bytes[i] = step_model_bytes(ex, ex->steps[i]); }
    return n;
}

extern "C" int ffgpu_exec_work_model(const ffgpu_exec *ex, double *hbm_bytes, double *flops)
{
    if (!ex || !ex->net) { ffgpu_set_error("work_model: bad executor"); return -1; }
    double by = 0, fl = 0;
    if (ex->child[0]) {
        for (int c = 0; c < ex->nchild; c++) {
            double b1 = 0, f1 = 0;
            if (ffgpu_exec_work_model(ex->child[c], &b1, &f1)) return -1;
            by += b1; fl += f1;
        }
    } else {
        const double N = ex->N;
        for (const Step &st : ex->steps) by += step_model_bytes(ex, st);
        const LAYER *ll = ex->net->layer_list;
        for (int i = 0; i < ex->net->layer_num; i++)
            if (ll[i].type == LAYER_TYPE_CONV)
                fl += 2.0 * N * ll[i].fs * ll[i].fs * (ll[i].c / ll[i].groups) * (double)ll[i + 1].c * ll[i + 1].w * ll[i + 1].h;
    }
    if (hbm_bytes) *hbm_bytes = by;
    if (flops) *flops = fl;
    return 0;
}

extern "C" int ffgpu_exec_set_scale(ffgpu_exec *ex, int s1, int s2)
{
    if (!ex || s2 == 0) { ffgpu_set_error("set_scale: bad arguments"); return -1; }
    ex->s1 = s1; ex->s2 = s2;
    return 0;
}

extern "C" int ffgpu_exec_forward_dev(ffgpu_exec *ex, const float *d_frames, void *stream)
{
    if (!alive(ex, "forward_dev")) return -1;
    if (!d_frames) { ffgpu_set_error("forward_dev: NULL argument"); return -1; }
    return forward_on(ex, fp32_src(d_frames), stream ? (hipStream_t)stream : ex->own_stream);
}

static int ensure_input(ffgpu_exec *ex)
{
    if (ex->d_input) return 0;
    FFGPU_CHECK(hipMalloc(&ex->d_input, sizeof(float) * (size_t)ex->N * ex->in_c * ex->in_h * ex->in_w));
    return 0;
}

extern "C" int ffgpu_exec_forward_host(ffgpu_exec *ex, const float *h_frames)
{
    if (!alive(ex, "forward_host")) return -1;
    if (!h_frames) { ffgpu_set_error("forward_host: NULL argument"); return -1; }
    if (ensure_input(ex)) return -1;
    const size_t bytes = sizeof(float) * (size_t)ex->N * ex->in_c * ex->in_h * ex->in_w;
    if (pinned_ours(h_frames, bytes)) {
        FFGPU_CHECK(hipMemcpyAsync(ex->d_input, h_frames, bytes, hipMemcpyHostToDevice, ex->own_stream));
    } else {
        if (!ex->h_stage) FFGPU_CHECK(hipHostMalloc((void **)&ex->h_stage, bytes, hipHostMallocDefault));
        memcpy(ex->h_stage, h_frames, bytes);
        FFGPU_CHECK(hipMemcpyAsync(ex->d_input, ex->h_stage, bytes, hipMemcpyHostToDevice, ex->own_stream));
    }
    if (forward_on(ex, fp32_src(ex->d_input), ex->own_stream)) return -1;
    FFGPU_CHECK(hipStreamSynchronize(ex->own_stream));
// ... 659 lines not shown
    for (ffgpu_exec *ex : dev->execs)
        if (repack(ex, stream ? (hipStream_t)stream : ex->own_stream)) return -1;
    if (!stream) for (ffgpu_exec *ex : dev->execs) FFGPU_CHECK(hipStreamSynchronize(ex->own_stream));
    return 0;
}

#include "ffgpu_node.inc"

static void fill_desc(ConvDesc &d, const float *in, const float *filt, float *out, int batch,
                      int iw, int ih, int ic, int groups, int pad, int stride, int fs, int ow, int oh, int oc, int act, int flags)
{
    memset(&d, 0, sizeof d);
    d.in = in; d.filt = filt; d.out = out; d.N = batch;
    d.iw = iw; d.ih = ih; d.ic = ic; d.ow = ow; d.oh = oh; d.oc = oc;
    d.fs = fs; d.stride = stride; d.pad = pad; d.groups = groups; d.act = act; d.flags = flags & (FFGPU_COMPAT_V6 | FFGPU_BF16_PW);
    d.in_cs = (long)batch * iw * ih; d.in_ns = (long)iw * ih;
    d.out_cs = (long)batch * ow * oh; d.out_ns = (long)ow * oh;
}

extern "C" int ffgpu_groupconv_dev(const float *d_in, const float *d_filt, float *d_out, int batch,
                                   int iw, int ih, int ic, int groups, int pad, int stride,
                                   int fs, int fn, int ow, int oh, int oc, int act,
                                   int flags, int variant, void *stream)
{
    if (!d_in || !d_filt || !d_out || batch < 1 || fn != oc) { ffgpu_set_error("groupconv_dev: bad arguments"); return -1; }
    ConvDesc d;
    fill_desc(d, d_in, d_filt, d_out, batch, iw, ih, ic, groups, pad, stride, fs, ow, oh, oc, act, flags);
    return ffgpu_launch_conv(d, variant, (hipStream_t)stream);
}

extern "C" const char *ffgpu_groupconv_kernel_name(int batch, int iw, int ih, int ic, int groups, int pad,
                                                   int stride, int fs, int fn, int variant)
{
    ConvDesc d;
    const int ow = (iw + 2 * pad - fs) / stride + 1, oh = (ih + 2 * pad - fs) / stride + 1;
    fill_desc(d, nullptr, nullptr, nullptr, batch, iw, ih, ic, groups, pad, stride, fs, ow, oh, fn, 0, 0);
    return ffgpu_conv_kernel_name(d, variant);
}

extern "C" float ffgpu_groupconv_time_dev(const float *d_in, const float *d_filt, float *d_out, int batch,
                                          int iw, int ih, int ic, int groups, int pad, int stride,
                                          int fs, int fn, int ow, int oh, int oc, int act,
                                          int flags, int variant, int warmup, int iters, void *stream)
{
    if (iters < 1 || fn != oc) { ffgpu_set_error("groupconv_time_dev: bad arguments"); return -1.f; }
    hipStream_t s = (hipStream_t)stream;
    ConvDesc d;
    fill_desc(d, d_in, d_filt, d_out, batch, iw, ih, ic, groups, pad, stride, fs, ow, oh, oc, act, flags);
    float *pk = nullptr;
    if (variant == FFGPU_K_AUTO && ffgpu_pw_pack_floats(d) > 0) {
        if (hipMalloc(&pk, ffgpu_pw_pack_floats(d) * sizeof(float)) != hipSuccess || ffgpu_pw_pack(d, pk, s)) { ffgpu_set_error("pack failed"); return -1.f; }
        d.wpack = pk;
    }
    hipEvent_t e0, e1;
    if (hipEventCreate(&e0) != hipSuccess || hipEventCreate(&e1) != hipSuccess) { ffgpu_set_error("hipEventCreate failed"); return -1.f; }
    for (int i = 0; i < warmup; i++) if (ffgpu_launch_conv(d, variant, s)) return -1.f;
    (void)hipEventRecord(e0, s);
    for (int i = 0; i < iters; i++) if (ffgpu_launch_conv(d, variant, s)) return -1.f;
    (void)hipEventRecord(e1, s);
    if (hipEventSynchronize(e1) != hipSuccess) { ffgpu_set_error("hipEventSynchronize: %s", hipGetErrorString(hipGetLastError())); return -1.f; }
    float ms = 0.f;
    (void)hipEventElapsedTime(&ms, e0, e1);
    (void)hipEventDestroy(e0); (void)hipEventDestroy(e1);
    return ms * 1000.f / iters;
}

static void irb_fill(IrbDesc &d, int batch, int iw, int ih, int ic, int ec, int oc, int stride, int act1, int actd, int act2, int res_act)
{
    d.N = batch; d.H = ih; d.W = iw; d.OH = (ih + 2 - 3) / stride + 1; d.OW = (iw + 2 - 3) / stride + 1;
    d.ic = ic; d.ec = ec; d.oc = oc; d.stride = stride;
    d.act1 = act1; d.actd = actd; d.act2 = act2; d.res_act = res_act;
}

extern "C" int ffgpu_irb_plan_text(int batch, int iw, int ih, int ic, int ec, int oc, int stride, int act1, int actd, int act2, int res_act, int flags, char *buf, int cap)
{
    if (!buf || cap < 1 || batch < 1 || iw < 1 || ih < 1 || stride < 1) { ffgpu_set_error("irb_plan_text: bad arguments"); return -1; }
    IrbDesc d{};
    irb_fill(d, batch, iw, ih, ic, ec, oc, stride, act1, actd, act2, res_act);
    d.flags = flags & FFGPU_CONCURRENT;
    (void)ffgpu_irb_plan(d);
    return ffgpu_irb_plan_line(d, buf, (size_t)cap);
}

extern "C" int ffgpu_irb_instantiations(char *buf, int cap)
{
    if (!buf || cap < 1) { ffgpu_set_error("irb_instantiations: bad arguments"); return -1; }
    return ffgpu_irb_keys(buf, (size_t)cap);
}

extern "C" int ffgpu_knobs_text(char *buf, int cap)
{
    if (!buf || cap < 1) { ffgpu_set_error("knobs_text: bad arguments"); return -1; }
    return ffgpu_knobs_lines(buf, (size_t)cap);
}

extern "C" float ffgpu_irb_dev(const float *d_in, const float *d_w1, const float *d_wd, const float *d_w2,
                               const float *d_res, float *d_out, int batch, int iw, int ih, int ic, int ec, int oc,
                               int stride, int act1, int actd, int act2, int res_act, int warmup, int iters, void *stream)
{
    hipStream_t s = (hipStream_t)stream;
    IrbDesc d{};
    d.in = d_in; d.out = d_out; d.residual = d_res; d.w1 = d_w1; d.wd = d_wd; d.w2 = d_w2;
    irb_fill(d, batch, iw, ih, ic, ec, oc, stride, act1, actd, act2, res_act);
    if (!d_in || !d_out || !d_w1 || !d_wd || !d_w2 || !ffgpu_irb_plan(d)) { ffgpu_set_error("irb_dev: unsupported block shape"); return -1.f; }
    float *pk = nullptr;
    if (hipMalloc(&pk, ffgpu_irb_pack_floats(d) * sizeof(float)) != hipSuccess) { ffgpu_set_error("irb_dev: hipMalloc failed"); return -1.f; }
    d.pk = pk;
    float us = 0.f;
    int rc = ffgpu_irb_pack(d, pk, s);
    if (!rc && iters <= 0) rc = ffgpu_launch_irb(d, s);
    if (!rc && iters > 0) {
        hipEvent_t e0, e1;
        (void)hipEventCreate(&e0); (void)hipEventCreate(&e1);
        for (int i = 0; i < warmup && !rc; i++) rc = ffgpu_launch_irb(d, s);
        (void)hipEventRecord(e0, s);
        for (int i = 0; i < iters && !rc; i++) rc = ffgpu_launch_irb(d, s);
        (void)hipEventRecord(e1, s);
        (void)hipEventSynchronize(e1);
        float ms = 0.f;
        (void)hipEventElapsedTime(&ms, e0, e1);
        us = ms * 1000.f / iters;
        (void)hipEventDestroy(e0); (void)hipEventDestroy(e1);
    }
    (void)hipStreamSynchronize(s);
    (void)hipFree(pk);
    return rc ? -1.f : us;
}

extern "C" float ffgpu_dwpw_dev(const float *d_in, const float *d_wd, const float *d_wp, float *d_out, int batch, int iw, int ih,
                                int c, int oc, int fs, int actd, int actp, int warmup, int iters, void *stream)
{
    hipStream_t s = (hipStream_t)stream;
    ConvDesc dw, pw;
    fill_desc(dw, d_in, d_wd, nullptr, batch, iw, ih, c, c, fs / 2, 1, fs, iw, ih, c, actd, 0);
    fill_desc(pw, nullptr, d_wp, d_out, batch, iw, ih, c, 1, 0, 1, 1, iw, ih, oc, actp, 0);
    if (!d_in || !d_wd || !d_wp || !d_out || !ffgpu_dwpw_ok(dw, pw)) { ffgpu_set_error("dwpw_dev: unsupported layer pair"); return -1.f; }
    float *pk = nullptr;
    if (hipMalloc(&pk, ffgpu_dwpw_pack_floats(dw, pw) * sizeof(float)) != hipSuccess) { ffgpu_set_error("dwpw_dev: hipMalloc failed"); return -1.f; }
    float us = 0.f;
    int rc = ffgpu_dwpw_pack(dw, pw, pk, s);
    if (!rc && iters <= 0) rc = ffgpu_launch_dwpw(dw, pw, pk, s);
    if (!rc && iters > 0) {
        hipEvent_t e0, e1;
        (void)hipEventCreate(&e0); (void)hipEventCreate(&e1);
        for (int i = 0; i < warmup && !rc; i++) rc = ffgpu_launch_dwpw(dw, pw, pk, s);
        (void)hipEventRecord(e0, s);
        for (int i = 0; i < iters && !rc; i++) rc = ffgpu_launch_dwpw(dw, pw, pk, s);
        (void)hipEventRecord(e1, s);
        (void)hipEventSynchronize(e1);
        float ms = 0.f;
        (void)hipEventElapsedTime(&ms, e0, e1);
        us = ms * 1000.f / iters;
        (void)hipEventDestroy(e0); (void)hipEventDestroy(e1);
    }
    (void)hipStreamSynchronize(s);
    (void)hipFree(pk);
    return rc ? -1.f : us;
}

struct HostConvScratch { float *in = nullptr, *filt = nullptr, *out = nullptr; size_t in_n = 0, filt_n = 0, out_n = 0; int dev = -1; };

static int grow(float **p, size_t *have, size_t need)
{
    if (*have >= need) return 0;
    (void)hipFree(*p);
    *p = nullptr; *have = 0;
// ... 30 lines not shown
```

ffcnn_amd/csrc/ffgpu_knobs.hpp:

```cpp
#pragma once
#include <assert.h>
#include <limits.h>
#include <stdio.h>
#include <stdlib.h>

enum KnobKind { KNOB_INT, KNOB_ON, KNOB_SET, KNOB_TEXT };
enum KnobClass { KNOB_PRODUCT, KNOB_TUNING, KNOB_TEST, KNOB_LAB };
#define KNOB_COMPUTED INT_MIN

#define FFGPU_KNOBS_MAIN(X) \
     \
    X(COMPAT_V6,         "FFCNN_COMPAT_V6",         ON,   0,             PRODUCT, "the reference's v6 behaviour for 5x5 filters (executors and groupconv)") \
    X(NO_GRAPH,          "FFGPU_NO_GRAPH",          ON,   0,             PRODUCT, "eager launches instead of a captured graph (as the flag FFGPU_NO_GRAPH)") \
    X(BF16_PW,           "FFGPU_BF16_PW",           ON,   0,             PRODUCT, "opt-in bf16 inputs for compute-bound pointwise layers; own tolerance (as the flag)") \
    X(NO_FUSE,           "FFGPU_NO_FUSE",           ON,   0,             PRODUCT, "one kernel per layer: no fused blocks, no concat in place, no residual in the conv epilogue (as the flag)") \
    X(BRANCH,            "FFGPU_BRANCH",            ON,   0,             PRODUCT, "first detection head as a parallel graph branch instead of in line") \
    X(DWPW,              "FFGPU_DWPW",              ON,   0,             PRODUCT, "the heads' depthwise + pointwise pairs as one kernel (measured slower)") \
    X(NO_U8_FRONT,       "FFGPU_NO_U8_FRONT",       SET,  0,             PRODUCT, "u8 frames through the staging kernel and the fp32 first kernel even where they could go straight in") \
    X(NV12_FRONT,        "FFGPU_NV12_FRONT",        INT,  KNOB_COMPUTED, PRODUCT, "1: NV12 frames into the NV12 form of k_front where the plan has it, 0: staged; default: the build's measured choice") \
    X(VERBOSE,           "FFGPU_VERBOSE",           SET,  0,             PRODUCT, "print every error to stderr as it is set") \
    X(NODE_PACK_BOXES,   "FFGPU_NODE_PACK_BOXES",   INT,  0,             PRODUCT, "room per frame in a shard's packed record block; 0 or less: 16, the constant of the same name in ffgpu_node.inc") \
    X(NO_IRB,            "FFGPU_NO_IRB",            ON,   0,             TUNING,  "no fused inverted-residual blocks: their three layers as three kernels") \
    X(IRB_MIN_EC,        "FFGPU_IRB_MIN_EC",        INT,  24,            TUNING,  "fewest expanded channels of a block the planner fuses (thin blocks apart)") \
    X(SPLIT_PARTS,       "FFGPU_SPLIT_PARTS",       INT,  2,             TUNING,  "parallel chains of an FFGPU_SPLIT2 executor: 2, 4 or 8 (where the batch divides)") \
    X(NO_INDIRECT,       "FFGPU_NO_INDIRECT",       ON,   0,             TEST,    "the first kernel takes the input address from its arguments, not the parameter block: graphs keyed by input pointer") \
     \
    X(FORCE_GENERIC,     "FFGPU_FORCE_GENERIC",     INT,  0,             PRODUCT, "the reference-order generic kernel for every convolution") \
    X(PW_X3,             "FFGPU_PW_X3",             INT,  1,             PRODUCT, "0: never pick the split-bf16 pointwise kernel k_pw_x3") \
    X(PWX3_MIN_IC,       "FFGPU_PWX3_MIN_IC",       INT,  192,           TUNING,  "k_pw_x3: fewest input channels AUTO takes it for") \
    X(PWX3_MIN_OC,       "FFGPU_PWX3_MIN_OC",       INT,  256,           TUNING,  "k_pw_x3: fewest output channels") \
    X(PWX3_MIN_P,        "FFGPU_PWX3_MIN_P",        INT,  65536,         TUNING,  "k_pw_x3: fewest pixels") \
    X(PWX3_MT,           "FFGPU_PWX3_MT",           INT,  0,             TUNING,  "k_pw_x3: 16-row blocks per wave, 1 / 2 / 4 (0: 4)") \
    X(PW_X3T,            "FFGPU_PW_X3T",            INT,  1,             PRODUCT, "0: never pick the tiled split-bf16 GEMM k_pw_x3t") \
    X(PWX3T_MIN_IC,      "FFGPU_PWX3T_MIN_IC",      INT,  128,           TUNING,  "k_pw_x3t: fewest input channels AUTO takes it for") \
    X(PWX3T_MIN_OC,      "FFGPU_PWX3T_MIN_OC",      INT,  192,           TUNING,  "k_pw_x3t: fewest output channels") \
    X(PWX3T_MIN_P,       "FFGPU_PWX3T_MIN_P",       INT,  65536,         TUNING,  "k_pw_x3t: fewest pixels") \
    X(PWXT_TM,           "FFGPU_PWXT_TM",           INT,  256,           TUNING,  "k_pw_x3t: channels per workgroup tile, 256 or 128 (frozen with a plan: ConvDesc::x3_mt)") \
    X(PWXT_NARROW,       "FFGPU_PWXT_NARROW",       INT,  1,             TUNING,  "k_pw_x3t: 0 switches the narrow tiles of the partial last round off") \
    X(PWXT_PERSIST,      "FFGPU_PWXT_PERSIST",      INT,  0,             TUNING,  "k_pw_x3t: persistent workgroups over the main tiles") \
    X(PWXT_NT,           "FFGPU_PWXT_NT",           INT,  -1,            TUNING,  "k_pw_x3t: non-temporal output stores never (0) / always (1); -1: outputs of 128 MB and more") \
    X(PWXT_DBG,          "FFGPU_PWXT_DBG",          INT,  0,             LAB,     "k_pw_x3t: ablation mask handed to the kernel (wrong results)") \
    X(PW_X3S,            "FFGPU_PW_X3S",            INT,  1,             PRODUCT, "0: never pick the pointwise form of k_conv_x3 (pw_x3s)") \
    X(PWX3S_MIN_IC,      "FFGPU_PWX3S_MIN_IC",      INT,  96,            TUNING,  "pw_x3s: fewest input channels AUTO takes it for") \
    X(PWX3S_MIN_OC,      "FFGPU_PWX3S_MIN_OC",      INT,  64,            TUNING,  "pw_x3s: fewest output channels") \
    X(PWX3S_MIN_WGS,     "FFGPU_PWX3S_MIN_WGS",     INT,  64,            TUNING,  "pw_x3s: fewest workgroups") \
    X(IG_X3,             "FFGPU_IG_X3",             INT,  1,             PRODUCT, "0: never pick the split-bf16 dense 3x3 kernel k_conv_x3") \
    X(IGX3_S2,           "FFGPU_IGX3_S2",           INT,  1,             TUNING,  "k_conv_x3: 0 keeps the stride-2 layers on the fp32 implicit GEMM") \
    X(IGX3_NW,           "FFGPU_IGX3_NW",           INT,  0,             TUNING,  "k_conv_x3: waves per workgroup, 4 or 8 (0: 8 at stride 2, else 4)") \
    X(IGX3_MT,           "FFGPU_IGX3_MT",           INT,  0,             TUNING,  "k_conv_x3: 16-row blocks per wave, 1 / 2 / 4 (0: by shape; frozen with a plan: ConvDesc::x3_mt)") \
    X(IGX3_MT4_WGS,      "FFGPU_IGX3_MT4_WGS",      INT,  192,           TUNING,  "k_conv_x3: fewest workgroups that four blocks per wave must leave") \
    X(IGX3_MIN_IC,       "FFGPU_IGX3_MIN_IC",       INT,  16,            TUNING,  "k_conv_x3: fewest input channels AUTO takes it for") \
    X(IGX3_MIN_WGS,      "FFGPU_IGX3_MIN_WGS",      INT,  160,           TUNING,  "k_conv_x3: fewest workgroups AUTO takes it for") \
    X(PWG_MIN_OC,        "FFGPU_PWG_MIN_OC",        INT,  128,           TUNING,  "k_pw_gemm32: fewest output channels AUTO takes it for") \
    X(PWG_MIN_IC,        "FFGPU_PWG_MIN_IC",        INT,  64,            TUNING,  "k_pw_gemm32: fewest input channels") \
    X(NO_PW_GEMM,        "FFGPU_NO_PW_GEMM",        INT,  0,             PRODUCT, "never pick k_pw_gemm32: k_pw_mfma instead") \
    X(NO_IGEMM,          "FFGPU_NO_IGEMM",          INT,  0,             TUNING,  "never pick the implicit GEMMs (k_conv_igemm, the dense form of k_conv_x3)") \
    X(NO_GROUP_THIN,     "FFGPU_NO_GROUP_THIN",     INT,  0,             TUNING,  "never pick k_conv_thin for grouped layers of few channels per group") \
    X(NO_DW_PAIR,        "FFGPU_NO_DW_PAIR",        INT,  0,             PRODUCT, "depthwise layers on k_dw_lds instead of k_dw_pair") \
    X(NO_CONV_FIRST,     "FFGPU_NO_CONV_FIRST",     INT,  0,             PRODUCT, "the first layer on the dense small-channel kernel instead of k_conv_first") \
    X(CONV_FIRST_MIN_PX, "FFGPU_CONV_FIRST_MIN_PX", INT,  262144,        TUNING,  "k_conv_first: fewest output pixels of the batch") \
    X(NO_POOL2X2,        "FFGPU_NO_POOL2X2",        INT,  0,             TEST,    "2x2 / stride 2 max pooling on the general pool kernel") \
     \
    X(IGEMM_NOVEC,       "FFGPU_IGEMM_NOVEC",       INT,  0,             TUNING,  "k_conv_igemm: no vector form of the gather") \
    X(IGEMM_SPLIT,       "FFGPU_IGEMM_SPLIT",       INT,  0,             TUNING,  "k_conv_igemm: split-K factor 1 .. 16 (0: by tile count; frozen with a plan: ConvDesc::nsplit)") \
    X(DW_U,              "FFGPU_DW_U",              INT,  4,             TUNING,  "k_dw3_stream: rows per step, 1 / 2 / 4") \
    X(DW_BAND,           "FFGPU_DW_BAND",           INT,  4,             TUNING,  "k_dw3_stream: rows per wave task (0: enough tasks to fill the chip)") \
    X(DW_NT,             "FFGPU_DW_NT",             INT,  -1,            PRODUCT, "k_dw3_stream: stream past the caches never (0) / always (1); -1: outputs of 128 MB and more") \
    X(DW_XCD,            "FFGPU_DW_XCD",            INT,  0,             TUNING,  "k_dw3_stream: walk the tasks XCD by XCD") \
    X(DWP_NI,            "FFGPU_DWP_NI",            INT,  0,             TUNING,  "k_dw_pair: frames per workgroup, at most (0: by shape)") \
    X(DWL_BH,            "FFGPU_DWL_BH",            INT,  0,             TUNING,  "k_dw_lds: rows per band (0: by shape)") \
    X(DWL_NPL,           "FFGPU_DWL_NPL",           INT,  0,             TUNING,  "k_dw_lds: planes per item (0: by shape)") \
    X(PWG_WM,            "FFGPU_PWG_WM",            INT,  0,             TUNING,  "k_pw_gemm32: waves per workgroup, 4 or 8 (0: 8 from 248 output channels; part of the packed image)") \
    X(PWG_NARROW,        "FFGPU_PWG_NARROW",        INT,  1,             TUNING,  "k_pw_gemm32: 0 switches the narrow tiles of the partial last round off") \
    X(PWG_DBG,           "FFGPU_PWG_DBG",           INT,  0,             LAB,     "k_pw_gemm32: ablation mask handed to the kernel (wrong results)") \
     \
    X(NO_THIN,           "FFGPU_NO_THIN",           INT,  0,             PRODUCT, "8-channel blocks on the wave kernel instead of k_irb_thin") \
    X(THIN_BAND,         "FFGPU_THIN_BAND",         INT,  KNOB_COMPUTED, TUNING,  "k_irb_thin: rows per wave; default by batch and height (thin_band)") \
    X(FRONT_BAND,        "FFGPU_FRONT_BAND",        INT,  KNOB_COMPUTED, TUNING,  "k_front: rows per wave; default as FFGPU_THIN_BAND") \
    X(NO_FRONT,          "FFGPU_NO_FRONT",          INT,  0,             PRODUCT, "layers 0-3 as k_conv_first + k_irb_thin instead of k_front") \
    X(FRONT_MIN_PX,      "FFGPU_FRONT_MIN_PX",      INT,  262144,        TUNING,  "k_front: fewest output pixels of the batch") \
    X(FRONT_NC,          "FFGPU_FRONT_NC",          INT,  3,             PRODUCT, "k_front: output columns per lane, 3 where a row fits a wave that way, or 4") \
    X(NO_IRBW,           "FFGPU_NO_IRBW",           INT,  0,             PRODUCT, "fused blocks on the workgroup kernel k_irb instead of the wave-autonomous k_irbw") \
    X(IRBW_S2_633,       "FFGPU_IRBW_S2_633",       INT,  1,             TUNING,  "k_irbw: 0 hides the stride-2 form for 24 input / 48 output channels from the planner") \
    X(IRBW_S2_NSI4,      "FFGPU_IRBW_S2_NSI4",      INT,  0,             TUNING,  "k_irbw: 1 lets the planner take the four-strip halo for the thin stride-2 blocks") \
    X(IRBW_TWQ,          "FFGPU_IRBW_TWQ",          INT,  0,             TUNING,  "k_irbw: tile width in quads (with FFGPU_IRBW_TH; 0: searched)") \
    X(IRBW_TH,           "FFGPU_IRBW_TH",           INT,  0,             TUNING,  "k_irbw: tile height (with FFGPU_IRBW_TWQ; 0: searched)") \
    X(IRBW_BIG,          "FFGPU_IRBW_BIG",          INT,  -1,            TUNING,  "k_irbw: the 256-register form never (0) / always (1); -1: by register need") \
    X(IRBW_BIG_S2K1,     "FFGPU_IRBW_BIG_S2K1",     INT,  -1,            TUNING,  "k_irbw: as FFGPU_IRBW_BIG for the stride-2 blocks of at most 4 input channels alone") \
    X(IRBW_GWAVES,       "FFGPU_IRBW_GWAVES",       INT,  KNOB_COMPUTED, TUNING,  "k_irbw: waves a launch wants before the group split stops; default 1200, 500 with FFGPU_CONCURRENT") \
    X(IRBW_NOEXC,        "FFGPU_IRBW_NOEXC",        INT,  0,             TUNING,  "k_irbw: without the measured exception (four waves on the 20x20 blocks)") \
    X(IRBW_G_MID,        "FFGPU_IRBW_G_MID",        INT,  0,             TUNING,  "k_irbw: group split for 256 .. 1099 tiles (0: as computed)") \
    X(IRBW_X3,           "FFGPU_IRBW_X3",           INT,  30,            PRODUCT, "fused blocks: expand GEMM as split-bf16 products, one bit per shape: 0: 8 input channels, 1: 16, 2: 24, 3: 48 (split tile in LDS), 4: the 40 -> 20 stride-2 block") \
    X(IRBW_G_XL,         "FFGPU_IRBW_G_XL",         INT,  7,             TUNING,  "k_irbw: group split of the LDS-resident form with several chains in flight") \
    X(IRBW_G_SMALL,      "FFGPU_IRBW_G_SMALL",      INT,  0,             TUNING,  "k_irbw: group split under 256 tiles (0: as computed)") \
    X(IRBW_G,            "FFGPU_IRBW_G",            INT,  0,             TUNING,  "k_irbw: group split, wins over everything (0: as computed)") \
    X(IRBW_NSO,          "FFGPU_IRBW_NSO",          INT,  2,             TUNING,  "k_irbw2: anything but 2 keeps the planner off the two-strip kernel") \
    X(IRBW2_TWQ,         "FFGPU_IRBW2_TWQ",         INT,  0,             TUNING,  "k_irbw2: tile width in quads (with FFGPU_IRBW2_TH; 0: searched)") \
    X(IRBW2_TH,          "FFGPU_IRBW2_TH",          INT,  0,             TUNING,  "k_irbw2: tile height (with FFGPU_IRBW2_TWQ; 0: searched)") \
    X(IRBW2_MIN_TILES,   "FFGPU_IRBW2_MIN_TILES",   INT,  768,           TUNING,  "k_irbw2: fewest tiles the planner takes it for") \
    X(IRBW_WPB,          "FFGPU_IRBW_WPB",          INT,  0,             TUNING,  "k_irbw: tiles per workgroup without a group split, 1 .. 8 (0: 4 or 8 by LDS)") \
    X(IRBW_HALF,         "FFGPU_IRBW_HALF",         INT,  1,             PRODUCT, "0: a last group of at most 8 real expanded channels is computed as a whole group") \
    X(IRBW_XCD,          "FFGPU_IRBW_XCD",          INT,  3,             PRODUCT, "fused blocks walk their tiles XCD by XCD; bit 0: one-wave-per-tile launches, bit 1: group-split launches") \
    X(IRBW_FOLD,         "FFGPU_IRBW_FOLD",         INT,  0,             TUNING,  "k_irbw: never widen the reduction region to all G partial sums (folding rounds)") \
    X(IRB_ECH,           "FFGPU_IRB_ECH",           INT,  0,             TUNING,  "k_irb: expanded channels per chunk, 16 or 32 (0: by shape)") \
    X(IRB_RESIDENT,      "FFGPU_IRB_RESIDENT",      INT,  1,             TUNING,  "k_irb: every chunk's constants in LDS never (0) / where it costs no workgroup (1) / wherever they fit (2)") \
    X(IRB_TW,            "FFGPU_IRB_TW",            INT,  0,             TUNING,  "k_irb: tile width (0: the measured table, then the search)") \
// ... 70 lines not shown
```

ffcnn_amd/csrc/ffgpu_plan.hpp:

```cpp
#pragma once
#include <algorithm>
#include <vector>
#include "ffcnn.h"

extern "C" void ffgpu_set_error(const char *fmt, ...);

struct Tensor {
    long size = 0;
    int  first = 1 << 30, last = -1;
    long off = -1;
    int  parent = -1;
    long parent_off = 0;
    bool used = false;
};

inline int root_of(const std::vector<Tensor> &ts, int t) { while (ts[t].parent >= 0) t = ts[t].parent; return t; }

struct PlanOptions {
    int  batch = 1;
    bool keep_all = false;
    bool fuse = true;
    bool branch = false;
    bool no_irb = false;
    int  irb_min_ec = 0;
    bool dwpw = false;
};

struct NetLayout {
    std::vector<Tensor> tensors;
    std::vector<int>    canon;
    std::vector<char>   readable;
    std::vector<char>   route_inplace;
    std::vector<int>    nuses;
    std::vector<int>    fused_into;
    std::vector<int>    irb_tail;
    std::vector<int>    dwpw_tail;
    int    side_lo = -1, side_hi = -1;
    size_t arena_floats = 0;

    int src(int i) const { return i < 0 ? -1 : canon[i]; }
    long offset_of(int t) const
    {
        long off = 0;
        while (tensors[t].parent >= 0) { off += tensors[t].parent_off; t = tensors[t].parent; }
        return tensors[t].off + off;
    }
};

template <class F>
void ffgpu_layer_reads(const LAYER *ll, const NetLayout &nl, int i, F f)
{
    if (ll[i].type != LAYER_TYPE_ROUTE) f(nl.src(i - 1));
    for (int k = 0; k < ll[i].depend_num; k++) f(nl.src(ll[i].depend_list[k]));
    if (nl.irb_tail[i] >= 0) f(nl.src(nl.irb_tail[i] - 1));
    if (nl.dwpw_tail[i] >= 0) f(nl.src(nl.dwpw_tail[i] - 1));
    if (nl.irb_tail[i] >= 0 && nl.fused_into[i] >= 0) f(nl.src(ll[nl.fused_into[i]].depend_list[0]));
}

inline void ffgpu_fold_onto_roots(std::vector<Tensor> &T)
{
    for (size_t t = 0; t < T.size(); t++) {
        if (!T[t].used || T[t].parent < 0) continue;
        Tensor &r = T[root_of(T, (int)t)];
        r.first = std::min(r.first, T[t].first);
        r.last = std::max(r.last, T[t].last);
    }
}

inline int ffgpu_layout_aliases(const LAYER *ll, int L, const PlanOptions &opt, NetLayout &nl)
{
    for (int i = 0; i < L; i++) {
        if (i > 0 && ll[i].type != LAYER_TYPE_ROUTE) nl.nuses[i - 1]++;
        for (int k = 0; k < ll[i].depend_num; k++) {
            const int d = ll[i].depend_list[k];
            if (d < 0 || d >= i) { ffgpu_set_error("layer %d depends on layer %d (not earlier)", i, d); return -1; }
            nl.nuses[d]++;
        }
    }
    for (int i = 0; i < L; i++) {
        switch (ll[i].type) {
        case LAYER_TYPE_DROPOUT: nl.canon[i] = nl.src(i - 1); break;
        case LAYER_TYPE_YOLO: nl.canon[i] = -2; break;
        case LAYER_TYPE_ROUTE:
            nl.canon[i] = (ll[i].depend_num == 1 && nl.src(ll[i].depend_list[0]) >= -1) ? nl.src(ll[i].depend_list[0]) : i;
            break;
        default: nl.canon[i] = i;
        }
        if (opt.fuse && ll[i].type == LAYER_TYPE_SHORTCUT && i > 0) {
            int p = i - 1;
            while (p > 0 && ll[p].type == LAYER_TYPE_DROPOUT && nl.nuses[p] == 1) p--;
            bool chain_private = ll[p].type == LAYER_TYPE_CONV && nl.nuses[p] == 1 && nl.src(ll[i].depend_list[0]) >= 0;
            for (int q = p + 1; q < i && chain_private; q++) chain_private = ll[q].type == LAYER_TYPE_DROPOUT && nl.nuses[q] == 1;
            if (chain_private) { nl.fused_into[p] = i; for (int q = p; q < i; q++) nl.canon[q] = i; }
        }
    }
    return 0;
}

template <class BlockOk>
void ffgpu_layout_irb(const LAYER *ll, int L, NetLayout &nl, BlockOk &&block_ok)
{
    for (int p0 = 0; p0 + 2 < L; p0++) {
        const LAYER &a = ll[p0], &b = ll[p0 + 1], &c = ll[p0 + 2];
        if (a.type != LAYER_TYPE_CONV || b.type != LAYER_TYPE_CONV || c.type != LAYER_TYPE_CONV) continue;
        const bool pw_a = a.fs == 1 && a.stride == 1 && a.pad == 0 && a.groups == 1;
        const bool dw_b = b.fs == 3 && b.pad == 1 && (b.stride == 1 || b.stride == 2) && b.groups == b.c && b.fn == b.c;
        const bool pw_c = c.fs == 1 && c.stride == 1 && c.pad == 0 && c.groups == 1;
        if (!pw_a || !dw_b || !pw_c || nl.nuses[p0] != 1 || nl.nuses[p0 + 1] != 1 || nl.src(p0 - 1) < 0) continue;
        if (nl.canon[p0] != p0 || nl.canon[p0 + 1] != p0 + 1) continue;
        if (!block_ok(p0)) continue;
        nl.irb_tail[p0 + 2] = p0;
        nl.canon[p0] = nl.canon[p0 + 1] = -3;
        p0 += 2;
    }
}

template <class PairOk>
void ffgpu_layout_dwpw(const LAYER *ll, int L, NetLayout &nl, PairOk &&pair_ok)
{
    for (int p0 = 0; p0 + 1 < L; p0++) {
        if (ll[p0].type != LAYER_TYPE_CONV || ll[p0 + 1].type != LAYER_TYPE_CONV) continue;
        if (nl.canon[p0] != p0 || nl.canon[p0 + 1] != p0 + 1 || nl.nuses[p0] != 1 || nl.fused_into[p0] >= 0 || nl.fused_into[p0 + 1] >= 0 || nl.src(p0 - 1) < 0) continue;
        if (!pair_ok(p0)) continue;
        nl.dwpw_tail[p0 + 1] = p0;
        nl.canon[p0] = -3;
        p0++;
    }
}

inline int ffgpu_layout_tensors(const LAYER *ll, int L, const PlanOptions &opt, NetLayout &nl)
{
    for (int i = 0; i < L; i++)
        if (nl.canon[i] == i) { nl.tensors[i].used = true; nl.tensors[i].size = (long)ll[i + 1].w * ll[i + 1].h * ll[i + 1].c * opt.batch; }
    for (int i = 0; i < L; i++) {
        if (nl.canon[i] == i) nl.readable[i] = 1;
        else if (ll[i].type == LAYER_TYPE_DROPOUT && i > 0 && nl.canon[i] >= 0 && nl.canon[i] == nl.canon[i - 1]) nl.readable[i] = nl.readable[i - 1];
        else if (ll[i].type == LAYER_TYPE_ROUTE && ll[i].depend_num == 1 && nl.canon[i] >= 0) nl.readable[i] = nl.readable[ll[i].depend_list[0]];
        for (int k = 0; ll[i].type == LAYER_TYPE_ROUTE && nl.canon[i] == i && k < ll[i].depend_num; k++) {
            const LAYER &o = ll[ll[i].depend_list[k] + 1];
            if (nl.src(ll[i].depend_list[k]) < 0 || (o.w == ll[i + 1].w && o.h == ll[i + 1].h)) continue;
            ffgpu_set_error("route %d: source layer %d is %d x %d, the route %d x %d", i, ll[i].depend_list[k], o.w, o.h, ll[i + 1].w, ll[i + 1].h);
            return -1;
        }
    }
    return 0;
}

inline void ffgpu_layout_concat(const LAYER *ll, int L, NetLayout &nl)
{
    std::vector<Tensor> &T = nl.tensors;
    for (int i = 0; i < L; i++) {
        if (ll[i].type != LAYER_TYPE_ROUTE || nl.canon[i] != i || ll[i].depend_num < 2) continue;
        bool ok = true;
        std::vector<int> kids;
        for (int k = 0; k < ll[i].depend_num && ok; k++) {
            const int t = nl.src(ll[i].depend_list[k]);
            ok = t >= 0 && T[t].parent < 0 && std::find(kids.begin(), kids.end(), t) == kids.end();
            kids.push_back(t);
        }
        if (!ok) continue;
        long off = 0;
        for (int t : kids) { T[t].parent = i; T[t].parent_off = off; off += T[t].size; }
        nl.route_inplace[i] = 1;
    }
}

inline void ffgpu_layout_lifetimes(const LAYER *ll, int L, NetLayout &nl)
{
    std::vector<Tensor> &T = nl.tensors;
    auto touch = [&](int t, int when) { if (t >= 0) { T[t].first = std::min(T[t].first, when); T[t].last = std::max(T[t].last, when); } };
    for (int i = 0; i < L; i++) {
        if (ll[i].type == LAYER_TYPE_DROPOUT) continue;
        if (nl.canon[i] >= 0 && !(ll[i].type == LAYER_TYPE_ROUTE && nl.canon[i] != i)) touch(nl.canon[i], i);
        ffgpu_layer_reads(ll, nl, i, [&](int t) { touch(t, i); });
    }
    ffgpu_fold_onto_roots(T);
}

inline void ffgpu_layout_side_lane(const LAYER *ll, int L, NetLayout &nl)
{
    std::vector<Tensor> &T = nl.tensors;
    for (int y = 0; y + 1 < L; y++) {
        if (ll[y].type != LAYER_TYPE_YOLO || ll[y + 1].type != LAYER_TYPE_ROUTE || ll[y + 1].depend_num != 1) continue;
        const int r = ll[y + 1].depend_list[0];
        bool ok = r >= 0 && r < y;
        for (int i = y + 1; i < L && ok; i++)
            for (int k = 0; k < ll[i].depend_num; k++) if (ll[i].depend_list[k] > r && ll[i].depend_list[k] <= y) ok = false;
        for (int i = r + 1; i <= y && ok; i++) if ((nl.irb_tail[i] >= 0 && nl.irb_tail[i] <= r) || (nl.dwpw_tail[i] >= 0 && nl.dwpw_tail[i] <= r)) ok = false;
        if (ok && nl.fused_into[r] > r) ok = false;
        if (!ok) continue;
        nl.side_lo = r + 1; nl.side_hi = y;
        for (int t = 0; t < L; t++) if (T[t].used && T[t].first > r) T[t].last = L + 1;
        for (int i = r + 1; i <= y; i++) ffgpu_layer_reads(ll, nl, i, [&](int t) { if (t >= 0) T[t].last = L + 1; });
        ffgpu_fold_onto_roots(T);
        break;
    }
}

inline void ffgpu_layout_arena(int L, const PlanOptions &opt, NetLayout &nl)
{
    std::vector<Tensor> &T = nl.tensors;
    struct Live { long off, size; int last; };
    std::vector<Live> live;
    long high = 0;
    std::vector<int> order;
    for (int t = 0; t < L; t++) if (T[t].used && T[t].parent < 0) order.push_back(t);
    std::sort(order.begin(), order.end(), [&](int a, int b) { return T[a].first != T[b].first ? T[a].first < T[b].first : a < b; });
    for (int t : order) {
        const long need = (T[t].size + 63) & ~63L;
        if (opt.keep_all) { T[t].off = high; high += need; continue; }
        live.erase(std::remove_if(live.begin(), live.end(), [&](const Live &l) { return l.last < T[t].first; }), live.end());
        std::sort(live.begin(), live.end(), [](const Live &a, const Live &b) { return a.off < b.off; });
        long at = 0;
        for (const Live &l : live) { if (at + need <= l.off) break; at = std::max(at, l.off + l.size); }
        T[t].off = at;
        live.push_back({ at, need, T[t].last });
        high = std::max(high, at + need);
    }
    nl.arena_floats = (size_t)std::max(high, 64L);
}

template <class BlockOk, class PairOk>
int ffgpu_net_layout(const LAYER *ll, int L, const PlanOptions &opt, BlockOk &&block_ok, PairOk &&pair_ok, NetLayout &nl)
{
    nl = NetLayout();
    nl.tensors.assign(L, Tensor());
    nl.canon.assign(L, -2);
    nl.readable.assign(L, 0); nl.route_inplace.assign(L, 0);
    nl.nuses.assign(L, 0);
    nl.fused_into.assign(L, -1); nl.irb_tail.assign(L, -1); nl.dwpw_tail.assign(L, -1);
    if (ffgpu_layout_aliases(ll, L, opt, nl)) return -1;
    if (opt.fuse && !opt.no_irb) ffgpu_layout_irb(ll, L, nl, block_ok);
    if (opt.fuse && opt.dwpw) ffgpu_layout_dwpw(ll, L, nl, pair_ok);
    if (ffgpu_layout_tensors(ll, L, opt, nl)) return -1;
    if (opt.fuse) ffgpu_layout_concat(ll, L, nl);
    ffgpu_layout_lifetimes(ll, L, nl);
    if (opt.fuse && opt.branch) ffgpu_layout_side_lane(ll, L, nl);
    ffgpu_layout_arena(L, opt, nl);
    return 0;
}
```

ffcnn_amd/csrc/san/plan_driver.cc:

```cpp
#include <stdio.h>
#include <stdlib.h>
#include <string.h>

#include "ffcnn.h"
#include "ffcnn_hip.h"
#include "../ffgpu_plan.hpp"

static int g_bad = 0;
#define VIOLATION(...) do { printf("VIOLATION " __VA_ARGS__); printf("\n"); g_bad = 1; } while (0)

static bool disjoint(const NetLayout &nl, int a, int b)
{
    const long a0 = nl.offset_of(a), a1 = a0 + nl.tensors[a].size, b0 = nl.offset_of(b), b1 = b0 + nl.tensors[b].size;
    return a1 <= b0 || b1 <= a0;
}

static void check(const LAYER *ll, int L, const PlanOptions &opt, const NetLayout &nl)
{
    const std::vector<Tensor> &T = nl.tensors;
    std::vector<int> roots;
    for (int t = 0; t < L; t++) if (T[t].used && T[t].parent < 0) roots.push_back(t);
    for (size_t x = 0; x < roots.size(); x++)
        for (size_t y = x + 1; y < roots.size(); y++) {
            const int a = roots[x], b = roots[y];
            const bool meet = T[a].first <= T[b].last && T[b].first <= T[a].last;
            if ((meet || opt.keep_all) && !disjoint(nl, a, b)) VIOLATION("I1: tensors %d and %d are live together and share arena space", a, b);
        }
    for (int t = 0; t < L; t++) {
        if (T[t].parent >= 0 && !(T[t].used && nl.route_inplace[T[t].parent] && T[T[t].parent].used)) VIOLATION("I2: tensor %d lies in %d, which is no concat in place", t, T[t].parent);
        if (!nl.route_inplace[t]) continue;
        long off = 0;
        for (int k = 0; k < ll[t].depend_num; k++) {
            const int c = nl.src(ll[t].depend_list[k]);
            if (c < 0 || T[c].parent != t || T[c].parent_off != off) { VIOLATION("I2: source %d of route %d is not at its place inside it", k, t); break; }
            off += T[c].size;
        }
        if (off != T[t].size) VIOLATION("I2: the sources of route %d have %ld floats, the route %ld", t, off, T[t].size);
        for (int c = 0; c < L; c++) {
            bool named = false;
            for (int k = 0; k < ll[t].depend_num; k++) named = named || nl.src(ll[t].depend_list[k]) == c;
            if (T[c].parent == t && !named) VIOLATION("I2: tensor %d lies in route %d, which does not name it", c, t);
        }
    }
    for (int i = 0; i < L; i++) {
        if (ll[i].type == LAYER_TYPE_DROPOUT) continue;
        auto live = [&](int t, const char *verb) {
            if (t < 0) return;
            const Tensor &r = T[root_of(T, t)];
            if (!T[t].used || T[t].first > i || T[t].last < i || r.first > i || r.last < i) VIOLATION("I3: layer %d %s tensor %d outside its lifetime %d .. %d", i, verb, t, T[t].first, T[t].last);
        };
        ffgpu_layer_reads(ll, nl, i, [&](int t) { live(t, "reads"); });
        if (nl.canon[i] >= 0 && !(ll[i].type == LAYER_TYPE_ROUTE && nl.canon[i] != i)) live(nl.canon[i], "writes");
    }
    for (int t = 0; t < L; t++) {
        if (!T[t].used) continue;
        if (T[t].size < 0 || nl.offset_of(t) < 0 || (size_t)(nl.offset_of(t) + T[t].size) > nl.arena_floats) VIOLATION("I4: tensor %d ends outside the arena", t);
        if (T[t].parent < 0 && T[t].off % 64) VIOLATION("I4: tensor %d starts at %ld, no multiple of 64 floats", t, T[t].off);
    }
    for (int i = 0; i < L; i++) if (nl.readable[i] && nl.canon[i] < 0) VIOLATION("I4: layer %d is readable without a tensor", i);
    if (nl.side_lo >= 0) {
        std::vector<char> kept(L, 0);
        for (int t = 0; t < L; t++) if (T[t].used && T[t].first >= nl.side_lo) kept[root_of(T, t)] = 1;
        for (int i = nl.side_lo; i <= nl.side_hi; i++) ffgpu_layer_reads(ll, nl, i, [&](int t) { if (t >= 0) kept[root_of(T, t)] = 1; });
        for (int a : roots)
            for (int b : roots)
                if (kept[a] && a != b && T[b].first >= T[a].first && !disjoint(nl, a, b)) VIOLATION("I5: tensor %d of the side lane shares arena space with the later tensor %d", a, b);
    }
}

int main(int argc, char **argv)
{
    if (argc != 7) { fprintf(stderr, "usage: %s cfg batch flags none|all dwpw branch\n", argv[0]); return 2; }
    const int flags = atoi(argv[3]);
    const bool take = !strcmp(argv[4], "all");
    PlanOptions opt;
    opt.batch = atoi(argv[2]);
    opt.keep_all = flags & FFGPU_KEEP_ALL; opt.fuse = !(flags & FFGPU_NO_FUSE);
    opt.dwpw = atoi(argv[5]) != 0; opt.branch = atoi(argv[6]) != 0;
    if (opt.batch < 1) { fprintf(stderr, "batch must be >= 1\n"); return 2; }
    NET *net = net_load(argv[1], NULL, 0, 0);
    if (!net) { printf("net_load: NULL (%s)\n", ffgpu_last_error()); return 0; }
    const LAYER *ll = net->layer_list;
    const int L = net->layer_num;
    NetLayout nl;
    if (ffgpu_net_layout(ll, L, opt, [&](int) { return take; }, [&](int) { return take; }, nl)) {
        printf("layout: refused (%s)\n", ffgpu_last_error());
        net_free(net);
        return 0;
    }
    int nfused = 0, nirb = 0, ndwpw = 0, ninplace = 0;
    for (int i = 0; i < L; i++) {
        const int c = nl.canon[i];
        if (c < 0) printf("%d %d %d - - - - -\n", i, c, (int)nl.readable[i]);
        else printf("%d %d %d %d %d %d %ld %ld\n", i, c, (int)nl.readable[i], nl.tensors[c].first, nl.tensors[c].last, root_of(nl.tensors, c), nl.offset_of(c), nl.tensors[c].size);
        nfused += nl.fused_into[i] >= 0; nirb += nl.irb_tail[i] >= 0; ndwpw += nl.dwpw_tail[i] >= 0; ninplace += nl.route_inplace[i] != 0;
    }
    printf("%d %d %zu\n", nl.side_lo, nl.side_hi, nl.arena_floats);
    printf("fused_into %d irb %d dwpw %d inplace %d\n", nfused, nirb, ndwpw, ninplace);
    check(ll, L, opt, nl);
    net_free(net);
    return g_bad;
}
```

include/ffcnn_hip.h:

```cpp
#ifndef FFCNN_AMD_FFCNN_HIP_H
#define FFCNN_AMD_FFCNN_HIP_H

#include <stddef.h>
#include "ffcnn.h"

#ifdef __cplusplus
extern "C" {
#endif

#define FFGPU_MAX_DET   128



typedef struct {
    int  count;
    int  ncand;
    int  overflow;
    int  nfull;
    BBOX box[FFGPU_MAX_DET];
} ffgpu_frame_dets;

typedef struct ffgpu_exec ffgpu_exec;

#define FFGPU_KEEP_ALL   1
// ... 53 lines not shown
    int pitch_y;
    int pitch_uv;
    int matrix;
    int reserved;
} ffgpu_nv12_frame;

int ffgpu_exec_forward_nv12_frames_dev(ffgpu_exec *ex, const ffgpu_nv12_frame *frames, int nframes,
                                       const float mean[3], const float norm[3], void *stream);

int ffgpu_exec_dets_dev(ffgpu_exec *ex, void **dev_ptr, size_t *bytes);
const ffgpu_frame_dets *ffgpu_exec_dets_host(ffgpu_exec *ex);
int ffgpu_exec_set_ring(ffgpu_exec *ex, void *dev_ring, int slots);
int ffgpu_exec_set_ring_strided(ffgpu_exec *ex, void *dev_ring, int slots, int slot_records);
int ffgpu_exec_read_dets(ffgpu_exec *ex, ffgpu_frame_dets *host_out, int max_frames);
int ffgpu_exec_read_boxes(ffgpu_exec *ex, int frame, BBOX *host_out, int cap);
int ffgpu_exec_cand_capacity(const ffgpu_exec *ex);
int ffgpu_exec_graph_captures(const ffgpu_exec *ex);

int ffgpu_exec_read_layer(ffgpu_exec *ex, int layer, int frame, float *host_out, size_t cap_floats);

int ffgpu_exec_hash_layers(ffgpu_exec *ex, unsigned long long *host_out, int cap);

int ffgpu_exec_profile(ffgpu_exec *ex, const float *d_frames, float us_by_kind[LAYER_TYPE_TOTOAL]);

int ffgpu_exec_profile_steps(ffgpu_exec *ex, const float *d_frames, int *layer_of, float *us, int cap);
int ffgpu_exec_step_model(const ffgpu_exec *ex, int *layer_of, double *hbm_bytes, int cap);

typedef struct ffgpu_node ffgpu_node;
#define FFGPU_NODE_LOOPBACK 1
#define FFGPU_NODE_DEPTH(n) (((n) & 0xf) << 8)

void        ffgpu_shard_range(int total, int rank, int world, int *lo, int *hi);
ffgpu_node *ffgpu_node_create(NET *net, int ndev, const int *devices, int global_batch, int exec_flags, int node_flags);
void        ffgpu_node_destroy(ffgpu_node *node);
int         ffgpu_node_ndev(const ffgpu_node *node);
int         ffgpu_node_shard(const ffgpu_node *node, int rank, int *lo, int *hi, int *device);
int         ffgpu_node_set_scale(ffgpu_node *node, int s1, int s2);
int         ffgpu_node_depth(const ffgpu_node *node);
int         ffgpu_node_rccl_ranks(const ffgpu_node *node);
float      *ffgpu_node_input_dev(ffgpu_node *node, int rank);
float      *ffgpu_node_input_slot_dev(ffgpu_node *node, int rank, int slot);
int         ffgpu_node_forward(ffgpu_node *node, ffgpu_frame_dets *host_out);
int         ffgpu_node_forward_host(ffgpu_node *node, const float *h_frames, ffgpu_frame_dets *host_out);
long        ffgpu_node_submit(ffgpu_node *node, const float *h_frames);
int         ffgpu_node_wait(ffgpu_node *node, long ticket, ffgpu_frame_dets *host_out);
int         ffgpu_node_run(ffgpu_node *node, long steps, ffgpu_frame_dets *host_out);

int ffgpu_groupconv_dev(const float *d_in, const float *d_filt, float *d_out, int batch,
                        int iw, int ih, int ic, int groups, int pad, int stride,
                        int fs, int fn, int ow, int oh, int oc, int act,
                        int flags, int variant, void *stream);

enum {
    FFGPU_K_AUTO = 0,
    FFGPU_K_GENERIC = 1,
    FFGPU_K_DW_STREAM = 2,
    FFGPU_K_DW_LDS = 3,
    FFGPU_K_PW_MFMA = 4,
    FFGPU_K_PW_GEMM = 5,
    FFGPU_K_DENSE_SMALL = 7,
    FFGPU_K_IGEMM = 8,
    FFGPU_K_PW_BF16 = 9,
    FFGPU_K_GROUP_THIN = 10,
    FFGPU_K_PW_X3 = 11,
    FFGPU_K_CONV_X3 = 12,
    FFGPU_K_PW_X3T = 13
};

const char *ffgpu_groupconv_kernel_name(int batch, int iw, int ih, int ic, int groups, int pad,
                                        int stride, int fs, int fn, int variant);

float ffgpu_groupconv_time_dev(const float *d_in, const float *d_filt, float *d_out, int batch,
                               int iw, int ih, int ic, int groups, int pad, int stride,
                               int fs, int fn, int ow, int oh, int oc, int act,
                               int flags, int variant, int warmup, int iters, void *stream);

float ffgpu_irb_dev(const float *d_in, const float *d_w1, const float *d_wd, const float *d_w2,
                    const float *d_res, float *d_out, int batch, int iw, int ih, int ic, int ec, int oc,
                    int stride, int act1, int actd, int act2, int res_act, int warmup, int iters, void *stream);

int ffgpu_irb_plan_text(int batch, int iw, int ih, int ic, int ec, int oc, int stride, int act1, int actd, int act2, int res_act,
                        int flags, char *buf, int cap);

int ffgpu_irb_instantiations(char *buf, int cap);

int ffgpu_knobs_text(char *buf, int cap);

float ffgpu_dwpw_dev(const float *d_in, const float *d_wd, const float *d_wp, float *d_out, int batch, int iw, int ih,
                     int c, int oc, int fs, int actd, int actp, int warmup, int iters, void *stream);

size_t ffgpu_packed_records_bytes(int batch, int cap);
int    ffgpu_unpack_records(const void *block, int batch, int cap, ffgpu_frame_dets *out);
int    ffgpu_pack_records(const void *d_records, int nslots, long slot_stride_records, int batch, int cap, void *d_out, void *stream);

typedef struct {
    int image;
    int x0, y0;
    int reserved;
} ffgpu_tile;

#define FFGPU_MERGE_LDS_SLOTS 1024

size_t ffgpu_merge_tiles_scratch_bytes(int ntiles, int list_stride);
int    ffgpu_merge_tiles_dev(const void *d_records, const void *d_lists, int list_stride, const ffgpu_tile *tiles, int ntiles, int nimages,
                             float thresh, int use_min, void *d_out_records, void *d_out_lists, void *d_scratch, size_t scratch_bytes, void *stream);

int ffgpu_exec_merge_tiles(ffgpu_exec *ex, const ffgpu_tile *tiles, int ntiles, int nimages, void *stream);
int ffgpu_exec_merged_dev(ffgpu_exec *ex, void **dev_ptr, size_t *bytes);
int ffgpu_exec_read_merged(ffgpu_exec *ex, ffgpu_frame_dets *host_out, int max_images);
int ffgpu_exec_read_merged_boxes(ffgpu_exec *ex, int image, BBOX *host_out, int cap);

typedef struct { int x0, y0, w, h; } ffgpu_tile_rect;
int ffgpu_tile_plan(int img_w, int img_h, int tile_w, int tile_h, int overlap_x, int overlap_y, int align, ffgpu_tile_rect *out, int cap);

typedef struct {
    unsigned char color[4];
    const unsigned char *palette;
    int npalette;
    int thickness;
} ffgpu_draw_style;

int ffgpu_draw_boxes_bgr_dev (const void *d_records, const void *d_lists, int list_stride, const int *list_first,
                              const ffgpu_bgr_frame  *targets, int ntargets, const ffgpu_draw_style *style, void *stream);
int ffgpu_draw_boxes_nv12_dev(const void *d_records, const void *d_lists, int list_stride, const int *list_first,
                              const ffgpu_nv12_frame *targets, int ntargets, const ffgpu_draw_style *style, void *stream);

#define FFGPU_DRAW_ENTRIES 0
#define FFGPU_DRAW_MERGED  1
int ffgpu_exec_draw_bgr (ffgpu_exec *ex, int which, const ffgpu_bgr_frame  *targets, int ntargets, const ffgpu_draw_style *style, void *stream);
int ffgpu_exec_draw_nv12(ffgpu_exec *ex, int which, const ffgpu_nv12_frame *targets, int ntargets, const ffgpu_draw_style *style, void *stream);

#define FFGPU_CROP_F32 0
#define FFGPU_CROP_U8  1
typedef struct {
    int   out_w, out_h;
    int   form;
    int   per_target;
    float min_score;
    int   nclasses;
    const unsigned char *classes;
    int   margin_num, margin_den;
    float mean[3], norm[3];
    int   reserved;
} ffgpu_crop_spec;
typedef struct {
    int   target, box, type;
    float score;
    int   x0, y0, w, h;
    int   sw, sh, s1, s2;
} ffgpu_crop;

size_t ffgpu_crop_table_bytes(int capacity);
size_t ffgpu_crop_slot_bytes(int out_w, int out_h, int form);

int ffgpu_crop_boxes_bgr_dev (const void *d_records, const void *d_lists, int list_stride, const int *list_first, const ffgpu_bgr_frame  *sources,
                              int ntargets, const ffgpu_crop_spec *spec, void *d_out, void *d_table, int capacity, void *stream);
int ffgpu_crop_boxes_nv12_dev(const void *d_records, const void *d_lists, int list_stride, const int *list_first, const ffgpu_nv12_frame *sources,
                              int ntargets, const ffgpu_crop_spec *spec, void *d_out, void *d_table, int capacity, void *stream);

#define FFGPU_CROP_ENTRIES 0
#define FFGPU_CROP_MERGED  1
int ffgpu_exec_crop_bgr (ffgpu_exec *ex, int which, const ffgpu_bgr_frame  *sources, int ntargets, const ffgpu_crop_spec *spec,
                         void *d_out, void *d_table, int capacity, void *stream);
int ffgpu_exec_crop_nv12(ffgpu_exec *ex, int which, const ffgpu_nv12_frame *sources, int ntargets, const ffgpu_crop_spec *spec,
                         void *d_out, void *d_table, int capacity, void *stream);

// ... 177 lines not shown
```

Before: 182,900.

## Fuse runs of identical inverted-residual blocks into one LDS-resident stage kernel

```diff
diff --git a/ffcnn_amd/capi.py b/ffcnn_amd/capi.py
--- a/ffcnn_amd/capi.py
+++ b/ffcnn_amd/capi.py
@@ -180,7 +180,7 @@
            "ffgpu_exec_kernel_count", "ffgpu_exec_work_model", "ffgpu_exec_set_scale", "ffgpu_exec_forward_dev", "ffgpu_exec_forward_host",
            "ffgpu_exec_forward_bgr_dev", "ffgpu_exec_forward_bgr_frames_dev", "ffgpu_exec_forward_nv12_frames_dev", "ffgpu_exec_dets_dev", "ffgpu_exec_dets_host", "ffgpu_exec_set_ring", "ffgpu_exec_set_ring_strided", "ffgpu_exec_read_dets", "ffgpu_exec_read_layer", "ffgpu_exec_hash_layers",
            "ffgpu_exec_read_boxes", "ffgpu_exec_cand_capacity", "ffgpu_exec_graph_captures",
-           "ffgpu_exec_profile", "ffgpu_exec_profile_steps", "ffgpu_exec_step_model", "ffgpu_groupconv_dev", "ffgpu_groupconv_kernel_name", "ffgpu_groupconv_time_dev", "ffgpu_irb_dev", "ffgpu_irb_plan_text", "ffgpu_irb_instantiations", "ffgpu_knobs_text", "ffgpu_dwpw_dev", "ffgpu_packed_records_bytes", "ffgpu_pack_records", "ffgpu_unpack_records",
+           "ffgpu_exec_profile", "ffgpu_exec_profile_steps", "ffgpu_exec_step_model", "ffgpu_groupconv_dev", "ffgpu_groupconv_kernel_name", "ffgpu_groupconv_time_dev", "ffgpu_irb_dev", "ffgpu_irb_plan_text", "ffgpu_irb_stage_plan_text", "ffgpu_irb_instantiations", "ffgpu_knobs_text", "ffgpu_dwpw_dev", "ffgpu_packed_records_bytes", "ffgpu_pack_records", "ffgpu_unpack_records",
            "ffgpu_shard_range", "ffgpu_node_create", "ffgpu_node_destroy", "ffgpu_node_ndev", "ffgpu_node_shard", "ffgpu_node_set_scale",
            "ffgpu_node_input_dev", "ffgpu_node_input_slot_dev", "ffgpu_node_depth", "ffgpu_node_rccl_ranks", "ffgpu_node_forward", "ffgpu_node_forward_host",
            "ffgpu_node_submit", "ffgpu_node_wait", "ffgpu_node_run",
@@ -270,6 +270,7 @@
     L.ffgpu_irb_dev.restype = C.c_float
     L.ffgpu_irb_dev.argtypes = [vp] * 6 + [i] * 13 + [vp]
     L.ffgpu_irb_plan_text.argtypes = [i] * 12 + [C.c_char_p, i]
+    L.ffgpu_irb_stage_plan_text.argtypes = [i] * 7 + [C.c_char_p, i]
     L.ffgpu_irb_instantiations.argtypes = [C.c_char_p, i]
     L.ffgpu_knobs_text.argtypes = [C.c_char_p, i]
     L.ffgpu_exec_read_boxes.argtypes = [vp, i, vp, i]
@@ -1165,6 +1166,13 @@
     return buf.value.decode()
 
 
+def irb_stage_plan_text(batch, iw, ih, blocks, act1=2, actd=2, flags=0):
+    buf = C.create_string_buffer(1024)
+    if lib().ffgpu_irb_stage_plan_text(batch, iw, ih, blocks, act1, actd, flags, buf, len(buf)) < 0:
+        raise RuntimeError("ffgpu_irb_stage_plan_text failed: %s" % last_error())
+    return buf.value.decode()
+
+
 def irb_instantiations():
     buf = C.create_string_buffer(4096)
     n = lib().ffgpu_irb_instantiations(buf, len(buf))
diff --git a/ffcnn_amd/csrc/ffgpu_conv_kernels.inc b/ffcnn_amd/csrc/ffgpu_conv_kernels.inc
--- a/ffcnn_amd/csrc/ffgpu_conv_kernels.inc
+++ b/ffcnn_amd/csrc/ffgpu_conv_kernels.inc
@@ -10,6 +10,7 @@
 #include "ffgpu_front.inc"
 #include "ffgpu_irb_wave.inc"
 #include "ffgpu_irb_wave2.inc"
+#include "ffgpu_irb_stage.inc"
 #include "ffgpu_pw_x3.inc"
 #include "ffgpu_pw_x3t.inc"
 #include "ffgpu_conv_x3.inc"
@@ -1528,3 +1529,64 @@
     if (!d.pk) { ffgpu_set_error("irb: constants not packed"); return -1; }
     return c.family == IRB_WAVE ? irbw_kernels[c.inst].launch(irbw_params(d), c, s) : irb_kernels[c.inst].launch(irb_params(d), c, s);
 }
+
+static bool irb_stage_params(const IrbDesc *blocks, int B, IrbStageP &p, size_t &lds)
+{
+    if (B < 2 || B > IRBS_MAXB) return false;
+    const IrbDesc &d0 = blocks[0];
+    for (int b = 0; b < B; b++) {
+        const IrbDesc &d = blocks[b];
+        const IrbPlan &c = d.plan;
+        if (d.ic != 48 || d.ec != 224 || d.oc != 48 || d.stride != 1 || d.OH != d.H || d.OW != d.W) return false;
+        if (d.N != d0.N || d.H != d0.H || d.W != d0.W || d.act1 != d0.act1 || d.actd != d0.actd) return false;
+        if (act_slope(d.act2) != 1.f || act_slope(d.res_act) != 1.f) return false;
+        if (c.family != IRB_WAVE || !c.xl || !c.x3 || c.half || c.G != IRBS_WAVES || c.KS1 != 12 || c.OT != 3 || c.ngroups != 2 * IRBS_WAVES) return false;
+        if (c.region / (c.OT * 1024) < c.G) return false;
+    }
+    const int plane = d0.H * d0.W, TWq = (d0.W + 3) / 4;
+    if (plane > 128 || TWq * d0.H > 32) return false;
+    p = IrbStageP{};
+    p.B = B; p.N = d0.N; p.H = d0.H; p.W = d0.W;
+    p.act1 = act_slope(d0.act1); p.actd = act_slope(d0.actd);
+    p.TWq = TWq; p.P = 4 * TWq + 2; p.EP = p.P * (d0.H + 2);
+    int total;
+    irbw_layout(d0.plan, p.o_w2, p.o_cs, p.cs_floats, total);
+    if (p.cs_floats > 2 * IRBS_WAVES * 64 * 4) return false;
+    p.e_off = p.cs_floats;
+    p.e_slice = std::max(16 * p.EP, 2048);
+    p.xi_off = p.e_off + IRBS_WAVES * p.e_slice;
+    p.f_off = p.xi_off + 2 * 4 * 64 * IRBW_XL_DW;
+    lds = (size_t)(p.f_off + 48 * plane) * sizeof(float);
+    p.m_w = umulhi_magic(d0.W); p.m_twq = umulhi_magic(TWq); p.m_plane = umulhi_magic(plane);
+    return lds <= IRB_LDS_MAX;
+}
+
+bool ffgpu_irb_stage_ok(const IrbDesc *blocks, int B)
+{
+    IrbStageP p; size_t lds;
+    return irb_stage_params(blocks, B, p, lds);
+}
+
+int ffgpu_irb_stage_line(const IrbDesc *blocks, int B, bool wanted, char *buf, size_t cap)
+{
+    IrbStageP p; size_t lds;
+    if (!wanted || !irb_stage_params(blocks, B, p, lds)) return snprintf(buf, cap, "blocks B=%d launches=%d", B, B);
+    return snprintf(buf, cap, "stage B=%d launches=1 N=%d H=%d W=%d act=%g,%g TWq=%d P=%d EP=%d o_w2=%d o_cs=%d cs_floats=%d e_off=%d e_slice=%d xi_off=%d f_off=%d m=%u,%u,%u lds=%zu grid=%d block=%d",
+                    p.B, p.N, p.H, p.W, p.act1, p.actd, p.TWq, p.P, p.EP, p.o_w2, p.o_cs, p.cs_floats, p.e_off, p.e_slice, p.xi_off, p.f_off, p.m_w, p.m_twq, p.m_plane, lds, p.N, IRBS_WAVES * 64);
+}
+
+int ffgpu_launch_irb_stage(const IrbDesc *blocks, int B, hipStream_t s)
+{
+    IrbStageP p; size_t lds;
+    if (!irb_stage_params(blocks, B, p, lds)) { ffgpu_set_error("irb_stage: the run of %d blocks does not fit the stage kernel", B); return -1; }
+    p.in = blocks[0].in; p.out = blocks[B - 1].out;
+    for (int b = 0; b < B; b++) {
+        if (!blocks[b].pk) { ffgpu_set_error("irb_stage: constants not packed"); return -1; }
+        p.pk[b] = blocks[b].pk;
+    }
+    if (!p.in || !p.out) { ffgpu_set_error("irb_stage: no tensors"); return -1; }
+    if (lds_allow((const void *)k_irb_stage, lds, "irb_stage")) return -1;
+    hipLaunchKernelGGL(k_irb_stage, dim3((unsigned)p.N), dim3(IRBS_WAVES * 64), lds, s, p);
+    LAUNCH_OK("irb_stage");
+    return 0;
+}
diff --git a/ffcnn_amd/csrc/ffgpu_dev.hpp b/ffcnn_amd/csrc/ffgpu_dev.hpp
--- a/ffcnn_amd/csrc/ffgpu_dev.hpp
+++ b/ffcnn_amd/csrc/ffgpu_dev.hpp
@@ -66,6 +66,10 @@
 int    ffgpu_launch_irb(const IrbDesc &d, hipStream_t s);
 int    ffgpu_irb_plan_line(const IrbDesc &d, char *buf, size_t cap);
 int    ffgpu_irb_keys(char *buf, size_t cap);
+#define IRBS_MAXB 8
+bool   ffgpu_irb_stage_ok(const IrbDesc *blocks, int B);
+int    ffgpu_launch_irb_stage(const IrbDesc *blocks, int B, hipStream_t s);
+int    ffgpu_irb_stage_line(const IrbDesc *blocks, int B, bool wanted, char *buf, size_t cap);
 bool   ffgpu_front_ok(const ConvDesc &c, const IrbDesc &d);
 enum InputForm { IN_F32, IN_U8, IN_BGR_FRAMES, IN_NV12_FRAMES, IN_FORMS };
 int    ffgpu_launch_front(const ConvDesc &c, const IrbDesc &d, InputForm form, hipStream_t s);
diff --git a/ffcnn_amd/csrc/ffgpu_exec.hip b/ffcnn_amd/csrc/ffgpu_exec.hip
--- a/ffcnn_amd/csrc/ffgpu_exec.hip
+++ b/ffcnn_amd/csrc/ffgpu_exec.hip
@@ -123,7 +123,7 @@
 
 #define FFGPU_INTERNAL_CHILD 0x40000000
 
-enum StepKind { S_CONV, S_POOL, S_UPSAMPLE, S_ADD, S_COPY, S_YOLO, S_NMS, S_CLEAR, S_TOCNHW, S_IRB, S_FRONT, S_DWPW };
+enum StepKind { S_CONV, S_POOL, S_UPSAMPLE, S_ADD, S_COPY, S_YOLO, S_NMS, S_CLEAR, S_TOCNHW, S_IRB, S_FRONT, S_DWPW, S_STAGE };
 
 struct Step {
     StepKind kind;
@@ -139,6 +139,7 @@
     int      w, h, c, fs, stride, flag;
     YoloHead head;
     IrbDesc  irb;
+    std::vector<IrbDesc> run;
     float   *out2[2];
     int      fs2[2];
     int      lane;
@@ -226,6 +227,11 @@
 
 static float *tensor_ptr(const ffgpu_exec *ex, int t) { return ex->arena + ex->layout.offset_of(t); }
 
+static bool stage_wanted(int N, int flags)
+{
+    return (flags & FFGPU_CONCURRENT) && !(flags & (FFGPU_KEEP_ALL | FFGPU_NO_FUSE)) && N >= 32 && knob(K_IRB_STAGE) != 0;
+}
+
 static PlanOptions plan_options(const ffgpu_exec *ex)
 {
     PlanOptions o;
@@ -235,6 +241,7 @@
     o.branch = knob(K_BRANCH) && !ex->is_child;
     o.no_irb = knob(K_NO_IRB); o.irb_min_ec = knob(K_IRB_MIN_EC);
     o.dwpw = knob(K_DWPW);
+    o.stage = stage_wanted(ex->N, ex->flags);
     return o;
 }
 
@@ -275,7 +282,13 @@
         return true;
     };
     auto pair_ok = [&](int p0) { return ffgpu_dwpw_ok(layer_desc(ex, p0), layer_desc(ex, p0 + 1)); };
-    return ffgpu_net_layout(ex->net->layer_list, ex->net->layer_num, opt, block_ok, pair_ok, ex->layout);
+    static_assert(FFGPU_STAGE_MAX_BLOCKS == IRBS_MAXB, "the layout's longest run is the stage kernel's");
+    auto run_ok = [&](const std::vector<int> &tails) {
+        std::vector<IrbDesc> run;
+        for (int t : tails) run.push_back(irb_planned[t]);
+        return ffgpu_irb_stage_ok(run.data(), (int)run.size());
+    };
+    return ffgpu_net_layout(ex->net->layer_list, ex->net->layer_num, opt, block_ok, pair_ok, run_ok, ex->layout);
 }
 
 static int plan_arena(ffgpu_exec *ex)
@@ -312,7 +325,17 @@
         switch (a.type) {
         case LAYER_TYPE_CONV: {
             if (nl.canon[i] == -3) break;
-            if (nl.irb_tail[i] >= 0) {
+            if (nl.stage_first[i] >= 0) {
+                st.kind = S_STAGE;
+                for (int t = nl.stage_first[i] + 2; t <= i; t++) {
+                    if (nl.irb_tail[t] < 0) continue;
+                    IrbDesc d = irb_planned[t];
+                    d.w1 = weights(nl.irb_tail[t]); d.wd = weights(nl.irb_tail[t] + 1); d.w2 = weights(nl.irb_tail[t] + 2);
+                    st.run.push_back(d);
+                }
+                st.run.front().in = ptr(nl.src(nl.stage_first[i] - 1));
+                st.run.back().out = ptr(nl.canon[i]);
+            } else if (nl.irb_tail[i] >= 0) {
                 const int p0 = nl.irb_tail[i];
                 IrbDesc &d = st.irb = irb_planned[i];
                 st.kind = S_IRB;
@@ -343,6 +366,8 @@
             S.push_back(st);
             break; }
         case LAYER_TYPE_AVGPOOL: case LAYER_TYPE_MAXPOOL: case LAYER_TYPE_UPSAMPLE: case LAYER_TYPE_SHORTCUT: {
+            if (nl.canon[i] == -3) break;
+            if (a.type == LAYER_TYPE_SHORTCUT && i > 0 && nl.canon[i - 1] == i) break;
             const float *src = in_ptr(i, &from_input);
             const bool b_input = a.type == LAYER_TYPE_SHORTCUT && nl.src(a.depend_list[0]) == -1;
             if (a.type == LAYER_TYPE_SHORTCUT && nl.src(a.depend_list[0]) < -1) { bad_chain = true; break; }
@@ -358,7 +383,6 @@
             st.in_is_input = from_input;
             st.a = src;
             if (a.type == LAYER_TYPE_SHORTCUT) {
-                if (nl.canon[i - 1] == i) break;
                 st.kind = S_ADD;
                 st.b = b_input ? cnhw_input : ptr(nl.src(a.depend_list[0]));
                 st.b_is_input = b_input && N == 1;
@@ -451,6 +475,7 @@
 static size_t pack_floats(const Step &st)
 {
     if (st.kind == S_IRB) return ffgpu_irb_pack_floats(st.irb);
+    if (st.kind == S_STAGE) { size_t n = 0; for (const IrbDesc &d : st.run) n += ffgpu_irb_pack_floats(d); return n; }
     if (st.kind == S_DWPW) return ffgpu_dwpw_pack_floats(st.conv, st.conv2);
     if (st.kind == S_CONV) return ffgpu_pw_pack_floats(st.conv);
     return 0;
@@ -472,6 +497,7 @@
     for (Step &st : ex->steps) {
         const size_t n = pack_floats(st);
         if (st.kind == S_IRB) st.irb.pk = ex->d_pack + off;
+        else if (st.kind == S_STAGE) { size_t o = off; for (IrbDesc &d : st.run) { d.pk = ex->d_pack + o; o += ffgpu_irb_pack_floats(d); } }
         else if (st.kind == S_DWPW) st.conv2.wpack = ex->d_pack + off;
         else if (st.kind == S_CONV && n) st.conv.wpack = ex->d_pack + off;
         off += n;
@@ -503,6 +529,7 @@
 {
     for (const Step &st : ex->steps) {
         if (st.kind == S_IRB && ffgpu_irb_pack(st.irb, const_cast<float *>(st.irb.pk), s)) return -1;
+        if (st.kind == S_STAGE) for (const IrbDesc &d : st.run) if (ffgpu_irb_pack(d, const_cast<float *>(d.pk), s)) return -1;
         if (st.kind == S_DWPW && ffgpu_dwpw_pack(st.conv, st.conv2, const_cast<float *>(st.conv2.wpack), s)) return -1;
         if (st.kind == S_CONV && st.conv.wpack && ffgpu_pw_pack(st.conv, const_cast<float *>(st.conv.wpack), s)) return -1;
     }
@@ -555,6 +582,8 @@
         return 0; }
     case S_IRB:
         return ffgpu_launch_irb(st.irb, s);
+    case S_STAGE:
+        return ffgpu_launch_irb_stage(st.run.data(), (int)st.run.size(), s);
     case S_DWPW:
         return ffgpu_launch_dwpw(st.conv, st.conv2, st.conv2.wpack, s);
     case S_FRONT: {
@@ -859,6 +888,8 @@
         return 4.0 * (N * d.ic * d.ih * d.iw + N * d.oc * d.oh * d.ow * (d.residual ? 2 : 1) + rows(d)); }
     case S_IRB: { const IrbDesc &d = st.irb;
         return 4.0 * (N * d.ic * d.H * d.W + N * d.oc * d.OH * d.OW * (d.residual ? 2 : 1) + (double)d.ec * (d.ic + 4 + 16) + (double)d.oc * (d.ec + 4)); }
+    case S_STAGE: { const IrbDesc &d = st.run.front();
+        return 4.0 * (N * d.ic * d.H * d.W + N * d.oc * d.OH * d.OW + (double)st.run.size() * ((double)d.ec * (d.ic + 4 + 16) + (double)d.oc * (d.ec + 4))); }
     case S_DWPW: { const ConvDesc &a = st.conv, &b = st.conv2;
         return 4.0 * (N * a.ic * a.ih * a.iw + N * b.oc * b.oh * b.ow + rows(a) + rows(b)); }
     case S_FRONT: { const ConvDesc &c = st.conv; const IrbDesc &d = st.irb;
@@ -1684,6 +1715,18 @@
     return ffgpu_irb_plan_line(d, buf, (size_t)cap);
 }
 
+extern "C" int ffgpu_irb_stage_plan_text(int batch, int iw, int ih, int blocks, int act1, int actd, int flags, char *buf, int cap)
+{
+    if (!buf || cap < 1 || batch < 1 || iw < 1 || ih < 1 || blocks < 1 || blocks > 64) { ffgpu_set_error("irb_stage_plan_text: bad arguments"); return -1; }
+    std::vector<IrbDesc> run((size_t)blocks, IrbDesc{});
+    for (IrbDesc &d : run) {
+        irb_fill(d, batch, iw, ih, 48, 224, 48, 1, act1, actd, 0, 0);
+        d.flags = flags & FFGPU_CONCURRENT;
+        if (!ffgpu_irb_plan(d)) return snprintf(buf, (size_t)cap, "unsupported");
+    }
+    return ffgpu_irb_stage_line(run.data(), blocks, stage_wanted(batch, flags), buf, (size_t)cap);
+}
+
 extern "C" int ffgpu_irb_instantiations(char *buf, int cap)
 {
     if (!buf || cap < 1) { ffgpu_set_error("irb_instantiations: bad arguments"); return -1; }
diff --git a/ffcnn_amd/csrc/ffgpu_irb_stage.inc b/ffcnn_amd/csrc/ffgpu_irb_stage.inc
--- /dev/null
+++ b/ffcnn_amd/csrc/ffgpu_irb_stage.inc
@@ -0,0 +1,277 @@
+template <int KS1> __device__ __forceinline__ void irbw_xl_split_px(bool xinf, const float (&v)[KS1], u4_w2 (&o)[5])
+{
+    unsigned b[3][KS1];
+    if (xinf) {
+#pragma unroll
+        for (int ks = 0; ks < KS1; ks++) {
+            const float r = x3_resid_t<true>(v[ks]), r2 = x3_resid2(r);
+            b[0][ks] = __float_as_uint(v[ks]); b[1][ks] = __float_as_uint(r); b[2][ks] = __float_as_uint(r2);
+        }
+    } else {
+#pragma unroll
+        for (int ks = 0; ks < KS1; ks++) {
+            const float r = x3_resid_t<false>(v[ks]), r2 = x3_resid2(r);
+            b[0][ks] = __float_as_uint(v[ks]); b[1][ks] = __float_as_uint(r); b[2][ks] = __float_as_uint(r2);
+        }
+    }
+#pragma unroll
+    for (int i = 0; i < IRBW_XL_DW; i++) {
+        const int pt = i < 18 ? i / 6 : 0, pr = i < 18 ? i % 6 : i - 14;
+        o[i >> 2][i & 3] = __builtin_amdgcn_perm(b[pt][2 * pr + 1], b[pt][2 * pr], 0x07060302u);
+    }
+}
+template <int NM> __device__ __forceinline__ void irbw_xl_expand2(const u4_w2 *src0, const u4_w2 *src1, const u4_w2 (&w1x)[NM], v4f_w &a0, v4f_w &a1)
+{
+    u4_w2 o[2][5];
+#pragma unroll
+    for (int i = 0; i < 5; i++) o[0][i] = src0[i];
+#pragma unroll
+    for (int i = 0; i < 5; i++) o[1][i] = src1[i];
+#pragma unroll
+    for (int m = 0; m < NM; m++) {
+        const v8bf_w2 A = __builtin_bit_cast(v8bf_w2, w1x[m]);
+        a0 = __builtin_amdgcn_mfma_f32_16x16x32_bf16(A, __builtin_bit_cast(v8bf_w2, o[0][irbw_xl_op(m)]), a0, 0, 0, 0);
+        a1 = __builtin_amdgcn_mfma_f32_16x16x32_bf16(A, __builtin_bit_cast(v8bf_w2, o[1][irbw_xl_op(m)]), a1, 0, 0, 0);
+    }
+}
+__device__ __forceinline__ v2f_w irbw_expand_act(v2f_w a, v2f_w sc, v2f_w bi, float act1, float fl_act1)
+{
+    const v2f_w t = a * sc + bi;
+    const v2f_w u = t * act1;
+    return (v2f_w){ act_max(t.x, u.x, fl_act1), act_max(t.y, u.y, fl_act1) };
+}
+struct IrbwTaps { v2f_w tap[9], sd, bd; };
+__device__ __forceinline__ void irbw_dw_taps(const float *wdp, IrbwTaps &k)
+{
+    v4f_w T[6];
+#pragma unroll
+    for (int i = 0; i < 6; i++) T[i] = *reinterpret_cast<const v4f_w *>(wdp + 4 * i);
+    k.tap[0] = (v2f_w){ T[0].x, T[0].y }; k.tap[1] = (v2f_w){ T[0].z, T[0].w }; k.tap[2] = (v2f_w){ T[1].x, T[1].y };
+    k.tap[3] = (v2f_w){ T[1].z, T[1].w }; k.tap[4] = (v2f_w){ T[2].x, T[2].y }; k.tap[5] = (v2f_w){ T[2].z, T[2].w };
+    k.tap[6] = (v2f_w){ T[3].x, T[3].y }; k.tap[7] = (v2f_w){ T[3].z, T[3].w }; k.tap[8] = (v2f_w){ T[4].x, T[4].y };
+    k.sd = (v2f_w){ T[4].z, T[4].w }; k.bd = (v2f_w){ T[5].x, T[5].y };
+}
+template <int S> __device__ __forceinline__ void irbw_dw_row(const IrbwTaps &k, int r, const v2f_w *x, v2f_w (&dv)[4])
+{
+#pragma unroll
+    for (int q = 0; q < 4; q++)
+#pragma unroll
+        for (int kx = 0; kx < 3; kx++) dv[q] += k.tap[r * 3 + kx] * x[S * q + kx];
+}
+__device__ __forceinline__ void irbw_dw_out(const IrbwTaps &k, const v2f_w (&dv)[4], float actd, float fl_actd, v2f_w (&bq)[4])
+{
+#pragma unroll
+    for (int q = 0; q < 4; q++) {
+        const v2f_w t = dv[q] * k.sd + k.bd;
+        const v2f_w u = t * actd;
+        bq[q] = (v2f_w){ act_max(t.x, u.x, fl_actd), act_max(t.y, u.y, fl_actd) };
+    }
+}
+template <int OT> __device__ __forceinline__ void irbw_project(v4f_w (&acc)[OT][4], const float (&w2)[4 * OT], int m, const v2f_w (&bq)[4])
+{
+#pragma unroll
+    for (int j = 0; j < 2; j++)
+#pragma unroll
+        for (int t = 0; t < OT; t++) {
+            const float a = w2[(2 * m + j) * OT + t];
+            acc[t][0] = __builtin_amdgcn_mfma_f32_16x16x4f32(a, j ? bq[0].y : bq[0].x, acc[t][0], 0, 0, 0);
+            acc[t][1] = __builtin_amdgcn_mfma_f32_16x16x4f32(a, j ? bq[1].y : bq[1].x, acc[t][1], 0, 0, 0);
+            acc[t][2] = __builtin_amdgcn_mfma_f32_16x16x4f32(a, j ? bq[2].y : bq[2].x, acc[t][2], 0, 0, 0);
+            acc[t][3] = __builtin_amdgcn_mfma_f32_16x16x4f32(a, j ? bq[3].y : bq[3].x, acc[t][3], 0, 0, 0);
+        }
+}
+
+#define IRBS_WAVES 7
+struct IrbStageP {
+    const float *in; float *out;
+    const float *pk[IRBS_MAXB];
+    int B, N, H, W;
+    float act1, actd;
+    int TWq, P, EP;
+    int o_w2, o_cs, cs_floats;
+    int e_off, e_slice, xi_off, f_off;
+    unsigned m_w, m_twq, m_plane;
+};
+
+__global__ void __launch_bounds__(IRBS_WAVES * 64, 2) k_irb_stage(IrbStageP p)
+{
+    constexpr int KS1 = 12, OT = 3, NM = irbw_x3_nm(KS1), G = IRBS_WAVES;
+    extern __shared__ __attribute__((aligned(16))) float smem[];
+    const int tid = threadIdx.x, wid = __builtin_amdgcn_readfirstlane(tid >> 6);
+    int lane = tid & 63, kq = lane >> 4, jq = lane & 15;
+    const int n = (int)blockIdx.x, plane = p.H * p.W, nstrips = (plane + 63) >> 6;
+    const float fl_act1 = act_floor(p.act1), fl_actd = act_floor(p.actd);
+    const int ecp = 14 * 16;
+    const float *Wd = smem, *Sb1 = smem + ecp * 12, *Sb2 = Sb1 + ecp * 2;
+    float *Ew = smem + p.e_off + wid * p.e_slice;
+    unsigned *XI = reinterpret_cast<unsigned *>(smem) + p.xi_off;
+    float *F = smem + p.f_off;
+    const v4f_w z = { 0.f, 0.f, 0.f, 0.f };
+    const int cs4 = p.cs_floats >> 2;
+
+    for (int i = tid; i < 48 * plane; i += G * 64) {
+        const int c = irbw_div(i, p.m_plane), px = i - c * plane;
+        F[i] = p.in[((long)c * p.N + n) * plane + px];
+    }
+    for (int i = tid; i < cs4; i += G * 64) reinterpret_cast<v4f_w *>(smem)[i] = irbw_ld<v4f_w>(p.pk[0], (unsigned)(p.o_cs + 4 * i) * 4u);
+
+    int ebase[2], fbase[2], nvalid[2];
+    const bool strip1 = p.TWq * p.H > 16;
+
+    struct W1T { u4_w2 x[NM]; };
+    W1T w1a;
+    float w2[4 * OT];
+    auto loadw1 = [&](const float *pk, int g) {
+#pragma unroll
+        for (int m = 0; m < NM; m++) w1a.x[m] = irbw_ld<u4_w2>(pk, (unsigned)((g * NM + m) * 64 + lane) * 16u);
+    };
+    auto loadw2 = [&](const float *pk, int g, float (&w)[4 * OT]) {
+#pragma unroll
+        for (int i = 0; i < 4 * OT; i++) w[i] = irbw_ld<float>(pk, (unsigned)(p.o_w2 + (g * 4 * OT + i) * 64 + lane) * 4u);
+    };
+    loadw1(p.pk[0], wid);
+
+    v4f_w acc[2][OT][4];
+    auto group = [&](const float *pk, int g, int gnext) {
+        loadw2(pk, g, w2);
+        __builtin_amdgcn_sched_barrier(0);
+        const float *sbp = Sb1 + (g * 4 + kq) * 8;
+        const v4f_w S4 = *reinterpret_cast<const v4f_w *>(sbp), B4 = *reinterpret_cast<const v4f_w *>(sbp + 4);
+        const v2f_w sc[2] = { { S4.x, S4.y }, { S4.z, S4.w } }, bi[2] = { { B4.x, B4.y }, { B4.z, B4.w } };
+#pragma unroll
+        for (int si = 0; si < 2; si++) {
+            if (si >= nstrips) break;
+            v4f_w a4[4] = { z, z, z, z };
+#pragma unroll
+            for (int qh = 0; qh < 2; qh++) {
+                const u4_w2 *src = reinterpret_cast<const u4_w2 *>(XI + ((si * 4 + 2 * qh) * 64 + lane) * IRBW_XL_DW);
+                irbw_xl_expand2<NM>(src, src + 64 * IRBW_XL_DW / 4, w1a.x, a4[2 * qh], a4[2 * qh + 1]);
+            }
+#pragma unroll
+            for (int q = 0; q < 4; q++) {
+                const int e = si * 64 + 4 * jq + q;
+                const int y = irbw_div(e, p.m_w), x = e - y * p.W;
+                if (e < plane) {
+                    float *dst = Ew + ((y + 1) * p.P + x + 1) * 2;
+#pragma unroll
+                    for (int rp = 0; rp < 2; rp++) {
+                        const v2f_w a = rp == 0 ? (v2f_w){ a4[q].x, a4[q].y } : (v2f_w){ a4[q].z, a4[q].w };
+                        *reinterpret_cast<v2f_w *>(dst + (2 * kq + rp) * p.EP * 2) = irbw_expand_act(a, sc[rp], bi[rp], p.act1, fl_act1);
+                    }
+                }
+            }
+        }
+        __builtin_amdgcn_sched_barrier(0);
+        if (gnext >= 0) loadw1(pk, gnext);
+#pragma unroll
+        for (int m = 0; m < 2; m++) {
+            const int pr = 2 * kq + m;
+            IrbwTaps k;
+            irbw_dw_taps(Wd + (g * 8 + pr) * 24, k);
+#pragma unroll
+            for (int so = 0; so < 2; so++) {
+                if (so == 1 && !strip1) break;
+                const float *ep = Ew + pr * p.EP * 2 + ebase[so];
+                v2f_w dv[4] = { { 0.f, 0.f }, { 0.f, 0.f }, { 0.f, 0.f }, { 0.f, 0.f } }, bq[4];
+#pragma unroll
+                for (int r = 0; r < 3; r++) {
+                    const float *row = ep + r * p.P * 2;
+                    v2f_w x[6];
+#pragma unroll
+                    for (int i = 0; i < 3; i++) {
+                        const v4f_w u = *reinterpret_cast<const v4f_w *>(row + 4 * i);
+                        x[2 * i] = (v2f_w){ u.x, u.y }; x[2 * i + 1] = (v2f_w){ u.z, u.w };
+                    }
+                    irbw_dw_row<1>(k, r, x, dv);
+                }
+                irbw_dw_out(k, dv, p.actd, fl_actd, bq);
+                irbw_project<OT>(acc[so], w2, m, bq);
+            }
+        }
+    };
+
+    for (int b = 0; b < p.B; b++) {
+        const float *pk = p.pk[b];
+        for (int i = lane; i < (p.e_slice >> 2); i += 64) reinterpret_cast<v4f_w *>(Ew)[i] = z;
+        lane = (tid & 63) + __float_as_int(Ew[0]); kq = lane >> 4; jq = lane & 15;
+#pragma unroll
+        for (int so = 0; so < 2; so++) {
+            const int j = so * 16 + jq, ty = irbw_div(j, p.m_twq), tq = j - ty * p.TWq;
+            const bool qv = ty < p.H;
+            ebase[so] = qv ? (ty * p.P + 4 * tq) * 2 : 0;
+            fbase[so] = qv ? ty * p.W + 4 * tq : 0;
+            nvalid[so] = qv ? min(4, p.W - 4 * tq) : 0;
+        }
+        if (b == 0) __syncthreads();
+        for (int item = wid; item < nstrips * 4; item += G) {
+            const int si = item >> 2, q = item & 3, e = si * 64 + 4 * jq + q;
+            float v[KS1];
+#pragma unroll
+            for (int ks = 0; ks < KS1; ks++) v[ks] = e < plane ? F[(4 * ks + kq) * plane + e] : 0.f;
+            float amax = 0.f;
+#pragma unroll
+            for (int ks = 0; ks < KS1; ks += 2) amax = x3_amax3(amax, v[ks], v[ks + 1]);
+            const bool xinf = X3_INF_X_FUSED && x3_wave_has_inf(amax);
+            u4_w2 o[5];
+            irbw_xl_split_px<KS1>(xinf, v, o);
+            u4_w2 *dst = reinterpret_cast<u4_w2 *>(XI + (item * 64 + lane) * IRBW_XL_DW);
+#pragma unroll
+            for (int i = 0; i < 5; i++) dst[i] = o[i];
+        }
+#pragma unroll
+        for (int so = 0; so < 2; so++)
+#pragma unroll
+            for (int t = 0; t < OT; t++)
+#pragma unroll
+                for (int q = 0; q < 4; q++) acc[so][t][q] = z;
+        __syncthreads();
+
+        group(pk, wid, wid + G);
+        group(pk, wid + G, -1);
+        __builtin_amdgcn_sched_barrier(0);
+
+        const bool more = b + 1 < p.B;
+        const float *pkn = p.pk[more ? b + 1 : b];
+        v4f_w cst[2];
+#pragma unroll
+        for (int u = 0; u < 2; u++) cst[u] = irbw_ld<v4f_w>(pkn, (unsigned)(p.o_cs + 4 * min(tid + u * G * 64, cs4 - 1)) * 4u);
+        loadw1(pkn, wid);
+
+#pragma unroll
+        for (int t = 0; t < OT; t++) {
+            if (t > 0) __syncthreads();
+#pragma unroll
+            for (int so = 0; so < 2; so++)
+#pragma unroll
+                for (int r = 0; r < 4; r++)
+                    *reinterpret_cast<v4f_w *>(Ew + ((so * 4 + r) * 64 + lane) * 4) = (v4f_w){ acc[so][t][0][r], acc[so][t][1][r], acc[so][t][2][r], acc[so][t][3][r] };
+            __syncthreads();
+            for (int row = wid; row < 8; row += G) {
+                const int so = row >> 2, r = row & 3;
+                if (so == 1 && !strip1) break;
+                const float *red = smem + p.e_off + (row * 64 + lane) * 4;
+                v4f_w v = *reinterpret_cast<const v4f_w *>(red);
+                for (int s = 1; s < G; s++) v += *reinterpret_cast<const v4f_w *>(red + s * p.e_slice);
+                const int o = 16 * t + 4 * kq + r;
+                v = pw_fma4_apart(v.x, v.y, v.z, v.w, Sb2[2 * o], Sb2[2 * o + 1]);
+                const int nv = so ? nvalid[1] : nvalid[0];
+                float *fp = F + o * plane + (so ? fbase[1] : fbase[0]);
+                float *gp = p.out + ((long)o * p.N + n) * plane + (so ? fbase[1] : fbase[0]);
+                if ((p.W & 3) == 0) {
+                    if (nv == 4) {
+                        v += *reinterpret_cast<const v4f_w *>(fp);
+                        if (more) *reinterpret_cast<v4f_w *>(fp) = v; else *reinterpret_cast<v4f_w *>(gp) = v;
+                    }
+                } else {
+#pragma unroll
+                    for (int q = 0; q < 4; q++)
+                        if (q < nv) { const float w = v[q] + fp[q]; if (more) fp[q] = w; else gp[q] = w; }
+                }
+            }
+        }
+        if (!more) break;
+        __syncthreads();
+#pragma unroll
+        for (int u = 0; u < 2; u++) if (tid + u * G * 64 < cs4) reinterpret_cast<v4f_w *>(smem)[tid + u * G * 64] = cst[u];
+    }
+}
diff --git a/ffcnn_amd/csrc/ffgpu_knobs.hpp b/ffcnn_amd/csrc/ffgpu_knobs.hpp
--- a/ffcnn_amd/csrc/ffgpu_knobs.hpp
+++ b/ffcnn_amd/csrc/ffgpu_knobs.hpp
@@ -22,6 +22,7 @@
     X(NODE_PACK_BOXES,   "FFGPU_NODE_PACK_BOXES",   INT,  0,             PRODUCT, "room per frame in a shard's packed record block; 0 or less: 16, the constant of the same name in ffgpu_node.inc") \
     X(NO_IRB,            "FFGPU_NO_IRB",            ON,   0,             TUNING,  "no fused inverted-residual blocks: their three layers as three kernels") \
     X(IRB_MIN_EC,        "FFGPU_IRB_MIN_EC",        INT,  24,            TUNING,  "fewest expanded channels of a block the planner fuses (thin blocks apart)") \
+    X(IRB_STAGE,         "FFGPU_IRB_STAGE",         INT,  1,             TUNING,  "runs of 48 -> 224 -> 48 blocks on a small plane as one launch in FFGPU_CONCURRENT executors of 32 frames or more (0: one launch per block)") \
     X(SPLIT_PARTS,       "FFGPU_SPLIT_PARTS",       INT,  2,             TUNING,  "parallel chains of an FFGPU_SPLIT2 executor: 2, 4 or 8 (where the batch divides)") \
     X(NO_INDIRECT,       "FFGPU_NO_INDIRECT",       ON,   0,             TEST,    "the first kernel takes the input address from its arguments, not the parameter block: graphs keyed by input pointer") \
      \
diff --git a/ffcnn_amd/csrc/ffgpu_plan.hpp b/ffcnn_amd/csrc/ffgpu_plan.hpp
--- a/ffcnn_amd/csrc/ffgpu_plan.hpp
+++ b/ffcnn_amd/csrc/ffgpu_plan.hpp
@@ -24,6 +24,7 @@
     bool no_irb = false;
     int  irb_min_ec = 0;
     bool dwpw = false;
+    bool stage = false;
 };
 
 struct NetLayout {
@@ -35,6 +36,8 @@
     std::vector<int>    fused_into;
     std::vector<int>    irb_tail;
     std::vector<int>    dwpw_tail;
+    std::vector<int>    stage_first;
+    std::vector<char>   stage_inner;
     int    side_lo = -1, side_hi = -1;
     size_t arena_floats = 0;
 
@@ -54,6 +57,7 @@
     for (int k = 0; k < ll[i].depend_num; k++) f(nl.src(ll[i].depend_list[k]));
     if (nl.irb_tail[i] >= 0) f(nl.src(nl.irb_tail[i] - 1));
     if (nl.dwpw_tail[i] >= 0) f(nl.src(nl.dwpw_tail[i] - 1));
+    if (nl.stage_first[i] >= 0) f(nl.src(nl.stage_first[i] - 1));
     if (nl.irb_tail[i] >= 0 && nl.fused_into[i] >= 0) f(nl.src(ll[nl.fused_into[i]].depend_list[0]));
 }
 
@@ -112,6 +116,50 @@
         nl.irb_tail[p0 + 2] = p0;
         nl.canon[p0] = nl.canon[p0 + 1] = -3;
         p0 += 2;
+    }
+}
+
+constexpr int FFGPU_STAGE_MAX_BLOCKS = 8;
+template <class RunOk>
+void ffgpu_layout_stage(const LAYER *ll, int L, NetLayout &nl, RunOk &&run_ok)
+{
+    auto linear = [](int act) { return act != 1 && act != 2 && act != 3; };
+    auto shaped = [&](int t) {
+        const int p0 = nl.irb_tail[t], s = nl.fused_into[t];
+        if (p0 < 0 || s < 0 || nl.canon[t] != s) return false;
+        const LAYER &a = ll[p0], &b = ll[p0 + 1], &c = ll[p0 + 2];
+        return a.c == 48 && a.fn == 224 && c.fn == 48 && b.stride == 1 && a.w * a.h <= 128 && (a.w + 3) / 4 * a.h <= 32 &&
+               linear(c.activation) && linear(ll[s].activation) && nl.src(ll[s].depend_list[0]) >= 0 && nl.src(ll[s].depend_list[0]) == nl.src(p0 - 1);
+    };
+    auto follows = [&](int t, int tn) {
+        const int out = nl.canon[t], p0n = nl.irb_tail[tn], sn = nl.fused_into[tn];
+        if (nl.src(p0n - 1) != out || ll[p0n].w != ll[nl.irb_tail[t]].w || ll[p0n].h != ll[nl.irb_tail[t]].h ||
+            ll[p0n].activation != ll[nl.irb_tail[t]].activation || ll[p0n + 1].activation != ll[nl.irb_tail[t] + 1].activation) return false;
+        for (int i = 0; i < L; i++) {
+            if (ll[i].type == LAYER_TYPE_DROPOUT || (i >= nl.irb_tail[t] && i <= out) || (i >= p0n && i <= sn)) continue;
+            bool reads = false;
+            ffgpu_layer_reads(ll, nl, i, [&](int x) { reads = reads || x == out; });
+            if (reads) return false;
+        }
+        return true;
+    };
+    for (int t = 0; t < L; t++) {
+        if (nl.irb_tail[t] < 0 || !shaped(t)) continue;
+        std::vector<int> run(1, t);
+        for (int tn = run.back() + 1; tn < L && (int)run.size() < FFGPU_STAGE_MAX_BLOCKS; tn++) {
+            if (nl.irb_tail[tn] < 0) continue;
+            if (!shaped(tn) || !follows(run.back(), tn)) break;
+            run.push_back(tn);
+        }
+        if (run.size() >= 2 && run_ok(run)) {
+            nl.stage_first[run.back()] = nl.irb_tail[run.front()];
+            for (size_t k = 0; k + 1 < run.size(); k++) {
+                const int out = nl.canon[run[k]];
+                nl.stage_inner[run[k]] = 1;
+                for (int i = 0; i < L; i++) if (nl.canon[i] == out) nl.canon[i] = -3;
+            }
+        }
+        t = run.back();
     }
 }
 
@@ -220,8 +268,8 @@
     nl.arena_floats = (size_t)std::max(high, 64L);
 }
 
-template <class BlockOk, class PairOk>
-int ffgpu_net_layout(const LAYER *ll, int L, const PlanOptions &opt, BlockOk &&block_ok, PairOk &&pair_ok, NetLayout &nl)
+template <class BlockOk, class PairOk, class RunOk>
+int ffgpu_net_layout(const LAYER *ll, int L, const PlanOptions &opt, BlockOk &&block_ok, PairOk &&pair_ok, RunOk &&run_ok, NetLayout &nl)
 {
     nl = NetLayout();
     nl.tensors.assign(L, Tensor());
@@ -229,8 +277,10 @@
     nl.readable.assign(L, 0); nl.route_inplace.assign(L, 0);
     nl.nuses.assign(L, 0);
     nl.fused_into.assign(L, -1); nl.irb_tail.assign(L, -1); nl.dwpw_tail.assign(L, -1);
+    nl.stage_first.assign(L, -1); nl.stage_inner.assign(L, 0);
     if (ffgpu_layout_aliases(ll, L, opt, nl)) return -1;
     if (opt.fuse && !opt.no_irb) ffgpu_layout_irb(ll, L, nl, block_ok);
+    if (opt.fuse && !opt.no_irb && !opt.keep_all && opt.stage) ffgpu_layout_stage(ll, L, nl, run_ok);
     if (opt.fuse && opt.dwpw) ffgpu_layout_dwpw(ll, L, nl, pair_ok);
     if (ffgpu_layout_tensors(ll, L, opt, nl)) return -1;
     if (opt.fuse) ffgpu_layout_concat(ll, L, nl);
@@ -239,3 +289,9 @@
     ffgpu_layout_arena(L, opt, nl);
     return 0;
 }
+
+template <class BlockOk, class PairOk>
+int ffgpu_net_layout(const LAYER *ll, int L, const PlanOptions &opt, BlockOk &&block_ok, PairOk &&pair_ok, NetLayout &nl)
+{
+    return ffgpu_net_layout(ll, L, opt, block_ok, pair_ok, [](const std::vector<int> &) { return false; }, nl);
+}
diff --git a/ffcnn_amd/csrc/san/plan_driver.cc b/ffcnn_amd/csrc/san/plan_driver.cc
--- a/ffcnn_amd/csrc/san/plan_driver.cc
+++ b/ffcnn_amd/csrc/san/plan_driver.cc
@@ -58,6 +58,12 @@
         if (T[t].parent < 0 && T[t].off % 64) VIOLATION("I4: tensor %d starts at %ld, no multiple of 64 floats", t, T[t].off);
     }
     for (int i = 0; i < L; i++) if (nl.readable[i] && nl.canon[i] < 0) VIOLATION("I4: layer %d is readable without a tensor", i);
+    for (int i = 0; i < L; i++) {
+        if (nl.stage_inner[i] && (nl.canon[i] != -3 || nl.irb_tail[i] < 0 || nl.fused_into[i] < 0 || T[nl.fused_into[i]].used)) VIOLATION("I6: layer %d ends a block inside a merged run and still has a tensor", i);
+        if (nl.stage_first[i] < 0) continue;
+        const int in = nl.src(nl.stage_first[i] - 1);
+        if (in < 0 || nl.canon[i] < 0 || T[in].last < i || !disjoint(nl, root_of(T, in), root_of(T, nl.canon[i]))) VIOLATION("I6: the run that ends at layer %d has no input of its own at its launch", i);
+    }
     if (nl.side_lo >= 0) {
         std::vector<char> kept(L, 0);
         for (int t = 0; t < L; t++) if (T[t].used && T[t].first >= nl.side_lo) kept[root_of(T, t)] = 1;
@@ -70,20 +76,21 @@
 
 int main(int argc, char **argv)
 {
-    if (argc != 7) { fprintf(stderr, "usage: %s cfg batch flags none|all dwpw branch\n", argv[0]); return 2; }
+    if (argc != 7 && argc != 8) { fprintf(stderr, "usage: %s cfg batch flags none|all dwpw branch [stage]\n", argv[0]); return 2; }
     const int flags = atoi(argv[3]);
     const bool take = !strcmp(argv[4], "all");
     PlanOptions opt;
     opt.batch = atoi(argv[2]);
     opt.keep_all = flags & FFGPU_KEEP_ALL; opt.fuse = !(flags & FFGPU_NO_FUSE);
     opt.dwpw = atoi(argv[5]) != 0; opt.branch = atoi(argv[6]) != 0;
+    opt.stage = argc == 8 && atoi(argv[7]) != 0;
     if (opt.batch < 1) { fprintf(stderr, "batch must be >= 1\n"); return 2; }
     NET *net = net_load(argv[1], NULL, 0, 0);
     if (!net) { printf("net_load: NULL (%s)\n", ffgpu_last_error()); return 0; }
     const LAYER *ll = net->layer_list;
     const int L = net->layer_num;
     NetLayout nl;
-    if (ffgpu_net_layout(ll, L, opt, [&](int) { return take; }, [&](int) { return take; }, nl)) {
+    if (ffgpu_net_layout(ll, L, opt, [&](int) { return take; }, [&](int) { return take; }, [&](const std::vector<int> &) { return take; }, nl)) {
         printf("layout: refused (%s)\n", ffgpu_last_error());
         net_free(net);
         return 0;
@@ -97,6 +104,12 @@
     }
     printf("%d %d %zu\n", nl.side_lo, nl.side_hi, nl.arena_floats);
     printf("fused_into %d irb %d dwpw %d inplace %d\n", nfused, nirb, ndwpw, ninplace);
+    for (int i = 0; i < L; i++) {
+        if (nl.stage_first[i] < 0) continue;
+        int blocks = 0;
+        for (int t = nl.stage_first[i] + 2; t <= i; t++) blocks += nl.irb_tail[t] >= 0;
+        printf("stage %d %d %d\n", nl.stage_first[i], i, blocks);
+    }
     check(ll, L, opt, nl);
     net_free(net);
     return g_bad;
diff --git a/include/ffcnn_hip.h b/include/ffcnn_hip.h
--- a/include/ffcnn_hip.h
+++ b/include/ffcnn_hip.h
@@ -159,6 +159,8 @@
 int ffgpu_irb_plan_text(int batch, int iw, int ih, int ic, int ec, int oc, int stride, int act1, int actd, int act2, int res_act,
                         int flags, char *buf, int cap);
 
+int ffgpu_irb_stage_plan_text(int batch, int iw, int ih, int blocks, int act1, int actd, int flags, char *buf, int cap);
+
 int ffgpu_irb_instantiations(char *buf, int cap);
 
 int ffgpu_knobs_text(char *buf, int cap);
```

Result: faster. 189,200 (median of 6 runs) (+3.5%).
